# facebookresearch/generative-recommenders

Hardware: NVIDIA H100
Metric: user-seqs/sec HSTU-large L=8192 d=256 bf16 fwd+bwd (higher is better)
Workload: dtype bf16

## Files before the change

generative_recommenders_b200/_lib.py:

```python
import ctypes as C
import os
from typing import Optional

import torch

_HERE = os.path.dirname(os.path.abspath(__file__))
LIB_PATH = os.environ.get("HSTU_B200_LIB") or os.path.join(_HERE, "lib", "libhstu_b200.so")

ABI_VERSION = 1
F32, BF16, F16, E4M3 = 0, 1, 2, 3
IMPL_AUTO, IMPL_GENERIC, IMPL_UMMA = 0, 1, 2

_DTYPES = {torch.float32: F32, torch.bfloat16: BF16, torch.float16: F16, torch.float8_e4m3fn: E4M3}


class AttnParams(C.Structure):
    _fields_ = [
        ("abi_version", C.c_int32), ("dtype", C.c_int32), ("impl", C.c_int32), ("batch", C.c_int32),
        ("heads", C.c_int32), ("dqk", C.c_int32), ("dv", C.c_int32), ("max_seq_len", C.c_int32),
        ("total_rows", C.c_int64), ("alpha", C.c_float), ("max_attn_len", C.c_int32),
        ("min_full_attn_seq_len", C.c_int32), ("contextual_seq_len", C.c_int32), ("delta_q_len", C.c_int32),
        ("offsets_are_i64", C.c_int32), ("num_targets_are_i64", C.c_int32),
        ("seq_offsets", C.c_void_p), ("num_targets", C.c_void_p), ("q", C.c_void_p), ("k", C.c_void_p),
        ("v", C.c_void_p), ("out", C.c_void_p),
        ("q_row_stride", C.c_int64), ("q_head_stride", C.c_int64), ("k_row_stride", C.c_int64),
        ("k_head_stride", C.c_int64), ("v_row_stride", C.c_int64), ("v_head_stride", C.c_int64),
        ("o_row_stride", C.c_int64), ("o_head_stride", C.c_int64),
        ("dout", C.c_void_p), ("dq", C.c_void_p), ("dk", C.c_void_p), ("dv_out", C.c_void_p),
        ("do_row_stride", C.c_int64), ("do_head_stride", C.c_int64), ("dq_row_stride", C.c_int64),
        ("dq_head_stride", C.c_int64), ("dk_row_stride", C.c_int64), ("dk_head_stride", C.c_int64),
        ("dv_row_stride", C.c_int64), ("dv_head_stride", C.c_int64),
        ("pos_w", C.c_void_p), ("ts_w", C.c_void_p), ("timestamps", C.c_void_p), ("num_ts_buckets", C.c_int32),
        ("deterministic", C.c_int32), ("dpos_w", C.c_void_p), ("dts_w", C.c_void_p),
        ("workspace", C.c_void_p), ("workspace_bytes", C.c_size_t),
    ]


class Descales(C.Structure):
    _fields_ = [
        ("q", C.c_void_p), ("k", C.c_void_p), ("v", C.c_void_p),
        ("q_batch_stride", C.c_int64), ("q_head_stride", C.c_int64), ("k_batch_stride", C.c_int64),
        ("k_head_stride", C.c_int64), ("v_batch_stride", C.c_int64), ("v_head_stride", C.c_int64),
    ]


class SslParams(C.Structure):
    _fields_ = [
        ("abi_version", C.c_int32), ("dtype", C.c_int32), ("N", C.c_int64), ("R", C.c_int32), ("D", C.c_int32),
        ("l2_norm", C.c_int32), ("l2_eps", C.c_float), ("temperature", C.c_float), ("reserved0", C.c_int32),
        ("q", C.c_void_p), ("pos_emb", C.c_void_p), ("table", C.c_void_p), ("pos_ids", C.c_void_p), ("neg_ids", C.c_void_p),
        ("logits", C.c_void_p), ("rnorm", C.c_void_p), ("lse", C.c_void_p), ("loss_rows", C.c_void_p),
        ("row_coef", C.c_void_p), ("d_q", C.c_void_p), ("d_pos_emb", C.c_void_p), ("d_table", C.c_void_p),
    ]


_lib: Optional[C.CDLL] = None

_i32, _i64, _f32, _u64, _vp = C.c_int32, C.c_int64, C.c_float, C.c_uint64, C.c_void_p

_PROTOS = {
    "hstu_last_error": (C.c_char_p, []),
    "hstu_abi_version": (C.c_int, []),
    "hstu_attn_workspace_bytes": (C.c_size_t, [C.POINTER(AttnParams), C.c_int]),
    "hstu_attn_fwd": (C.c_int, [C.POINTER(AttnParams), _vp]),
    "hstu_attn_bwd": (C.c_int, [C.POINTER(AttnParams), _vp]),
    "hstu_attn_fwd_fp8": (C.c_int, [C.POINTER(AttnParams), C.POINTER(Descales), _vp]),
    "hstu_attn_select_impl": (C.c_int, [C.POINTER(AttnParams), C.c_int]),
    "hstu_mask_valid": (C.c_int, [_i32] * 7),
    "hstu_kv_range_for_q_rows": (C.c_int, [_i32] * 7 + [C.POINTER(_i32)] * 2),
    "hstu_q_range_for_kv_rows": (C.c_int, [_i32] * 7 + [C.POINTER(_i32)] * 3),
    "hstu_layer_norm_fwd": (C.c_int, [_vp, _vp, _vp, _vp, _vp, _vp, _i64, _i32, _i64, _i64, _f32, _i32, _i32, _vp]),
    "hstu_layer_norm_bwd": (C.c_int, [_vp] * 10 + [_i64, _i32, _i64, _i64, _i64, _i32, _i32, _vp]),
    "hstu_norm_bwd_partial_rows": (_i32, []),
    "hstu_rms_norm_fwd": (C.c_int, [_vp, _vp, _vp, _vp, _i64, _i32, _f32, _i32, _vp]),
    "hstu_rms_norm_bwd": (C.c_int, [_vp] * 7 + [_i64, _i32, _i32, _vp]),
    "hstu_norm_mul_dropout_fwd": (C.c_int, [_vp] * 7 + [_i64, _i32, _i32, _i64, _i64, _f32, _f32, _u64, _i32, _i32, _i32, _i32, _vp]),
    "hstu_norm_mul_dropout_bwd": (C.c_int, [_vp] * 12 + [_i64, _i32, _i32, _i64, _i64, _i64, _i64, _f32, _u64, _i32, _i32, _i32, _i32, _vp]),
    "hstu_silu_fwd": (C.c_int, [_vp, _vp, _i64, _i32, _i64, _i64, _i32, _vp]),
    "hstu_silu_bwd": (C.c_int, [_vp, _vp, _vp, _i64, _i32, _i64, _i64, _i64, _i32, _vp]),
    "hstu_jagged_concat": (C.c_int, [_vp] * 5 + [_i32] * 8 + [_vp]),
    "hstu_jagged_split": (C.c_int, [_vp] * 5 + [_i32] * 8 + [_vp]),
    "hstu_position_embeddings_fwd": (C.c_int, [_vp] * 10 + [_i64, _i32, _i32, _i32, _i32, _i32, _f32, _i32, _i32, _i32, _i32, _i32, _i32, _vp]),
    "hstu_position_embeddings_bwd": (C.c_int, [_vp] * 6 + [_i64, _i32, _f32, _i32, _vp]),
    "hstu_jagged_dense_bmm_broadcast_add": (C.c_int, [_vp] * 5 + [_i32] * 7 + [_vp]),
    "hstu_jagged_dense_bmm_wgrad": (C.c_int, [_vp] * 5 + [_i32] * 6 + [_vp]),
    "hstu_sampled_softmax_fwd": (C.c_int, [C.POINTER(SslParams), _vp]),
    "hstu_sampled_softmax_bwd": (C.c_int, [C.POINTER(SslParams), _vp]),
}

EXPORTED_SYMBOLS = tuple(_PROTOS.keys())


def lib() -> C.CDLL:
    global _lib
    if _lib is None:
        if not os.path.exists(LIB_PATH):
            raise RuntimeError(
                f"{LIB_PATH} is missing: build it with `python -m generative_recommenders_b200.build` "
                "(there is no CPU / eager fallback for HammerKernel.CUDA)"
            )
        l = C.CDLL(LIB_PATH)
        for name, (res, args) in _PROTOS.items():
            fn = getattr(l, name)
            fn.restype = res
            fn.argtypes = args
        if l.hstu_abi_version() != ABI_VERSION:
            raise RuntimeError("libhstu_b200.so ABI version mismatch")
        _lib = l
    return _lib


_selftest: Optional[C.CDLL] = None


def selftest_lib() -> C.CDLL:
    global _selftest
    if _selftest is None:
        path = os.path.join(_HERE, "lib", "libhstu_b200_selftest.so")
        if not os.path.exists(path):
            raise RuntimeError(f"{path} is missing: build it with `python -m generative_recommenders_b200.build`")
        l = C.CDLL(path)
        l.hstu_umma_selftest.restype = C.c_int
        l.hstu_umma_selftest.argtypes = [C.c_char_p, C.c_size_t]
        _selftest = l
    return _selftest


LAUNCHES = 0
_TIMED = None


def note_launch(n: int = 1) -> None:
    global LAUNCHES
    LAUNCHES += n


def enable_timing(on: bool) -> None:
    global _TIMED
    _TIMED = {} if on else None


def timed_events():
    return _TIMED


class timed:

    def __init__(self, name: str, device):
        self.name, self.device = name, device

    def __enter__(self):
        if _TIMED is not None:
            self.e0 = torch.cuda.Event(enable_timing=True)
            self.e1 = torch.cuda.Event(enable_timing=True)
            self.e0.record(torch.cuda.current_stream(self.device))
        return self

    def __exit__(self, *exc):
        if _TIMED is not None:
            self.e1.record(torch.cuda.current_stream(self.device))
            _TIMED.setdefault(self.name, []).append((self.e0, self.e1))
        return False


def check(rc: int, what: str) -> None:
    if rc != 0:
        msg = lib().hstu_last_error().decode(errors="replace")
        raise RuntimeError(f"{what} failed (code {rc}): {msg}")


def dtype_code(t: torch.Tensor) -> int:
    try:
        return _DTYPES[t.dtype]
    except KeyError:
        raise RuntimeError(f"unsupported dtype {t.dtype} for the CUDA HSTU kernels") from None


def ptr(t: Optional[torch.Tensor]) -> Optional[int]:
    return None if t is None else t.data_ptr()


def stream_ptr(device: torch.device) -> int:
    return torch.cuda.current_stream(device).cuda_stream


def require_cuda(*tensors: Optional[torch.Tensor]) -> torch.device:
    dev = None
    for t in tensors:
        if t is None:
            continue
        if not t.is_cuda:
            raise RuntimeError("HammerKernel.CUDA ops need CUDA tensors (no CPU fallback)")
        if dev is None:
            dev = t.device
        elif t.device != dev:
            raise RuntimeError("all tensors must be on the same CUDA device")
    assert dev is not None
    return dev
```

generative_recommenders_b200/csrc/api.cu:

```cuda
#include <stdarg.h>
#include <string.h>

#include "common.cuh"
#include "internal.h"

namespace hstu {

static thread_local char g_err[512] = "";

void set_error(const char* fmt, ...) {
  va_list ap;
  va_start(ap, fmt);
  vsnprintf(g_err, sizeof(g_err), fmt, ap);
  va_end(ap);
}

static int validate_attn(const hstu_attn_params* p, bool bwd) {
  HSTU_CHECK_ARG(p != nullptr, "params is NULL");
  HSTU_CHECK_ARG(p->abi_version == HSTU_B200_ABI_VERSION, "ABI version mismatch: caller %d, library %d", p->abi_version,
                 HSTU_B200_ABI_VERSION);
  HSTU_CHECK_ARG(p->dtype == HSTU_F32 || p->dtype == HSTU_BF16 || p->dtype == HSTU_F16 || p->dtype == HSTU_E4M3, "bad dtype %d",
                 p->dtype);
  HSTU_CHECK_ARG(p->max_seq_len > 0, "max_seq_len must be larger than 0");
  HSTU_CHECK_ARG(p->batch >= 0 && p->heads > 0, "bad batch/heads");
  HSTU_CHECK_ARG(p->dqk > 0 && p->dv > 0 && p->dqk <= 256 && p->dv <= 256, "head dims must be in [1, 256] (dqk=%d, dv=%d)",
                 p->dqk, p->dv);
  HSTU_CHECK_ARG(p->total_rows >= 0, "negative total_rows");
  HSTU_CHECK_ARG(p->max_attn_len >= 0 && p->contextual_seq_len >= 0 && p->min_full_attn_seq_len >= 0, "negative mask option");
  if (p->batch == 0 || p->total_rows == 0) return 0;
  HSTU_CHECK_ARG(p->seq_offsets != nullptr, "seq_offsets is NULL");
  HSTU_CHECK_ARG(p->q && p->k && p->v, "q/k/v is NULL");
  if (!bwd) HSTU_CHECK_ARG(p->out != nullptr, "out is NULL");
  if (bwd) {
    HSTU_CHECK_ARG(p->dout && p->dq && p->dk && p->dv_out, "dout/dq/dk/dv is NULL");
    HSTU_CHECK_ARG(p->delta_q_len == 0, "backward of delta-q attention is not defined by the reference");
  }
  if (p->ts_w) HSTU_CHECK_ARG(p->timestamps != nullptr, "ts_w given without timestamps");
  HSTU_CHECK_ARG(p->impl >= HSTU_IMPL_AUTO && p->impl <= HSTU_IMPL_UMMA, "bad impl %d", p->impl);
  HSTU_CHECK_ARG(p->deterministic == 0 || p->deterministic == 1, "deterministic must be 0 or 1 (got %d)", p->deterministic);
  return 0;
}

int bind_device(const void* ptr) {
  if (ptr == nullptr) return 0;
  cudaPointerAttributes attr;
  cudaError_t e = cudaPointerGetAttributes(&attr, ptr);
  if (e != cudaSuccess || (attr.type != cudaMemoryTypeDevice && attr.type != cudaMemoryTypeManaged)) {
    cudaGetLastError();
    set_error("expected a CUDA device pointer (got %p: %s)", ptr, e == cudaSuccess ? "host memory" : cudaGetErrorString(e));
    return HSTU_ERR_INVALID_ARGUMENT;
  }
  HSTU_CUDA_OK(cudaSetDevice(attr.device));
  return 0;
}

static int select_impl(const hstu_attn_params* p, bool bwd) {
  if (p->dtype == HSTU_E4M3) {
    if (bwd) {
      set_error("fp8 (e4m3) attention has no backward: hstu_attn_fwd_fp8 is a forward-only entry");
      return HSTU_ERR_UNSUPPORTED;
    }
    if (p->impl == HSTU_IMPL_GENERIC) {
      set_error("fp8 (e4m3) attention runs on the wgmma kernels only: the generic kernels take no fp8 input");
      return HSTU_ERR_UNSUPPORTED;
    }
    if (int e = e4m3_fwd_check(*p)) return e;
    return HSTU_IMPL_UMMA;
  }
  if (bwd && p->deterministic && (p->pos_w != nullptr || p->ts_w != nullptr)) {
    set_error("deterministic backward with a relative bias is not supported: the dpos_w / dts_w gradients are added "
              "with atomics");
    return HSTU_ERR_UNSUPPORTED;
  }
  const bool can = wgmma_supported(*p, bwd);
  if (p->impl == HSTU_IMPL_GENERIC) return HSTU_IMPL_GENERIC;
  if (p->impl == HSTU_IMPL_UMMA) {
    if (!can) {
      set_error("wgmma path does not support this problem (dtype=%d dqk=%d dv=%d delta=%d bias=%d)", p->dtype, p->dqk,
                p->dv, p->delta_q_len, p->pos_w != nullptr || p->ts_w != nullptr);
      return HSTU_ERR_UNSUPPORTED;
    }
    return HSTU_IMPL_UMMA;
  }
  return can ? HSTU_IMPL_UMMA : HSTU_IMPL_GENERIC;
}

static int validate_descales(const hstu_attn_descales* d) {
  if (d == nullptr) return 0;
  const float* ptr[3] = {d->q, d->k, d->v};
  const int64_t bs[3] = {d->q_batch_stride, d->k_batch_stride, d->v_batch_stride};
  const int64_t hs[3] = {d->q_head_stride, d->k_head_stride, d->v_head_stride};
  for (int i = 0; i < 3; ++i) {
    const char name = "qkv"[i];
    HSTU_CHECK_ARG(bs[i] >= 0 && hs[i] >= 0, "%c descale: negative stride (batch %lld, head %lld)", name, (long long)bs[i],
                   (long long)hs[i]);
    HSTU_CHECK_ARG((reinterpret_cast<uintptr_t>(ptr[i]) & 3) == 0, "%c descale: %p is not a float pointer", name, (const void*)ptr[i]);
  }
  return 0;
}

static int check_descale_devices(const hstu_attn_descales* d) {
  if (d == nullptr) return 0;
  int dev = 0;
  HSTU_CUDA_OK(cudaGetDevice(&dev));
  const float* ptr[3] = {d->q, d->k, d->v};
  for (int i = 0; i < 3; ++i) {
    if (ptr[i] == nullptr) continue;
    cudaPointerAttributes attr;
    const cudaError_t e = cudaPointerGetAttributes(&attr, ptr[i]);
    if (e != cudaSuccess || (attr.type != cudaMemoryTypeDevice && attr.type != cudaMemoryTypeManaged) || attr.device != dev) {
      cudaGetLastError();
      set_error("%c descale: expected device memory of CUDA device %d (got %p)", "qkv"[i], dev, (const void*)ptr[i]);
      return HSTU_ERR_INVALID_ARGUMENT;
    }
  }
  return 0;
}

}

using namespace hstu;

extern "C" {

const char* hstu_last_error(void) { return g_err; }
int hstu_abi_version(void) { return HSTU_B200_ABI_VERSION; }

int hstu_attn_select_impl(const hstu_attn_params* p, int is_backward) {
  if (int e = validate_attn(p, is_backward != 0)) return e;
  return select_impl(p, is_backward != 0);
}

size_t hstu_attn_workspace_bytes(const hstu_attn_params* p, int is_backward) {
  if (p == nullptr) return 0;
  if (validate_attn(p, is_backward != 0) != 0) return 0;
  if (p->batch == 0 || p->total_rows == 0) return 0;
  int impl = select_impl(p, is_backward != 0);
  if (p->dtype == HSTU_E4M3) return impl == HSTU_IMPL_UMMA ? e4m3_v_copy_bytes(*p) : 0;
  if (impl == HSTU_IMPL_UMMA) return wgmma_workspace_bytes(*p, is_backward != 0);
  return 0;
}

int hstu_attn_fwd(const hstu_attn_params* p, void* stream) {
  if (int e = validate_attn(p, false)) return e;
  HSTU_CHECK_ARG(p->dtype != HSTU_E4M3, "hstu_attn_fwd: fp8 (e4m3) inputs go through hstu_attn_fwd_fp8 (with their descales)");
  if (p->batch == 0 || p->total_rows == 0) return 0;
  if (int e = bind_device(p->q)) return e;
  int impl = select_impl(p, false);
  if (impl < 0) return impl;
  if (impl == HSTU_IMPL_UMMA) return attn_wgmma_fwd(*p, (cudaStream_t)stream);
  return attn_generic_fwd(*p, (cudaStream_t)stream);
}

int hstu_attn_bwd(const hstu_attn_params* p, void* stream) {
  if (int e = validate_attn(p, true)) return e;
  if (p->dtype == HSTU_E4M3) {
    set_error("hstu_attn_bwd: fp8 (e4m3) attention has no backward (hstu_attn_fwd_fp8 is forward only)");
    return HSTU_ERR_UNSUPPORTED;
  }
  if (p->batch == 0 || p->total_rows == 0) return 0;
  if (int e = bind_device(p->q)) return e;
  int impl = select_impl(p, true);
  if (impl < 0) return impl;
  if (impl == HSTU_IMPL_UMMA) return attn_wgmma_bwd(*p, (cudaStream_t)stream);
  return attn_generic_bwd(*p, (cudaStream_t)stream);
}

int hstu_attn_fwd_fp8(const hstu_attn_params* p, const hstu_attn_descales* descales, void* stream) {
  if (int e = validate_attn(p, false)) return e;
  HSTU_CHECK_ARG(p->dtype == HSTU_E4M3, "hstu_attn_fwd_fp8: q, k, v must be HSTU_E4M3 (got dtype %d)", p->dtype);
  if (int e = validate_descales(descales)) return e;
  const int impl = select_impl(p, false);
  if (impl < 0) return impl;
  if (p->batch == 0 || p->total_rows == 0) return 0;
  if (int e = bind_device(p->q)) return e;
  if (int e = check_descale_devices(descales)) return e;
  if (!is_sm90()) {
    set_error("hstu_attn_fwd_fp8: the fp8 kernels need an sm_90 device");
    return HSTU_ERR_UNSUPPORTED;
  }
  hstu_attn_descales none;
  memset(&none, 0, sizeof(none));
  return attn_wgmma_fwd_e4m3(*p, descales ? *descales : none, (cudaStream_t)stream);
}

int hstu_mask_valid(int32_t len, int32_t num_targets, int32_t max_attn_len, int32_t min_full_attn_seq_len,
                    int32_t contextual_seq_len, int32_t i, int32_t j) {
  SeqMask m = make_seq_mask(len, num_targets, max_attn_len, min_full_attn_seq_len, contextual_seq_len);
  return mask_valid(m, i, j) ? 1 : 0;
}

int hstu_kv_range_for_q_rows(int32_t len, int32_t num_targets, int32_t max_attn_len, int32_t min_full_attn_seq_len,
                             int32_t contextual_seq_len, int32_t m0, int32_t m1, int32_t* lo, int32_t* hi) {
  HSTU_CHECK_ARG(lo && hi && m0 >= 0 && m1 > m0 && m1 <= len, "bad row range");
  SeqMask m = make_seq_mask(len, num_targets, max_attn_len, min_full_attn_seq_len, contextual_seq_len);
  int l, h;
  kv_range_for_q_rows(m, m0, m1, &l, &h);
  *lo = l;
  *hi = h;
  return 0;
}

int hstu_q_range_for_kv_rows(int32_t len, int32_t num_targets, int32_t max_attn_len, int32_t min_full_attn_seq_len,
                             int32_t contextual_seq_len, int32_t n0, int32_t n1, int32_t* lo, int32_t* hi,
                             int32_t* ctx_hi) {
  HSTU_CHECK_ARG(lo && hi && ctx_hi && n0 >= 0 && n1 > n0 && n1 <= len, "bad row range");
  SeqMask m = make_seq_mask(len, num_targets, max_attn_len, min_full_attn_seq_len, contextual_seq_len);
  int l, h, c;
  q_range_for_kv_rows(m, n0, n1, &l, &h, &c);
  *lo = l;
  *hi = h;
  *ctx_hi = c;
  return 0;
}

int hstu_layer_norm_fwd(const void* x, const void* w, const void* b, void* y, float* mean, float* rstd, int64_t n_rows,
                        int32_t D, int64_t x_row_stride, int64_t y_row_stride, float eps, int32_t dtype, int32_t swish,
                        void* stream) {
  if (n_rows > 0) if (int e = bind_device(x)) return e;
  HSTU_CHECK_ARG(n_rows >= 0 && (n_rows == 0 || (x && y)), "layer_norm_fwd: NULL x/y");
  return layer_norm_fwd(x, w, b, y, mean, rstd, n_rows, D, x_row_stride, y_row_stride, eps, dtype, swish, false,
                        (cudaStream_t)stream);
}

int hstu_layer_norm_bwd(const void* dy, const void* x, const void* w, const void* b, const float* mean, const float* rstd,
                        void* dx, float* dw, float* db, float* partial, int64_t n_rows, int32_t D, int64_t x_row_stride,
                        int64_t dy_row_stride, int64_t dx_row_stride, int32_t dtype, int32_t swish, void* stream) {
  if (n_rows > 0) if (int e = bind_device(x)) return e;
  HSTU_CHECK_ARG(n_rows >= 0 && (n_rows == 0 || (dy && x && dx && mean && rstd)), "layer_norm_bwd: NULL argument");
  return layer_norm_bwd(dy, x, w, b, mean, rstd, dx, dw, db, partial, n_rows, D, x_row_stride, dy_row_stride,
                        dx_row_stride, dtype, swish, false, (cudaStream_t)stream);
}

int32_t hstu_norm_bwd_partial_rows(void) { return norm_partial_rows(); }

int hstu_rms_norm_fwd(const void* x, const void* w, void* y, float* rstd, int64_t n_rows, int32_t D, float eps,
                      int32_t dtype, void* stream) {
  if (n_rows > 0) if (int e = bind_device(x)) return e;
  HSTU_CHECK_ARG(n_rows >= 0 && (n_rows == 0 || (x && y && w)), "rms_norm_fwd: NULL argument");
  return layer_norm_fwd(x, w, nullptr, y, nullptr, rstd, n_rows, D, D, D, eps, dtype, 0, true, (cudaStream_t)stream);
}

int hstu_rms_norm_bwd(const void* dy, const void* x, const void* w, const float* rstd, void* dx, float* dw,
                      float* partial, int64_t n_rows, int32_t D, int32_t dtype, void* stream) {
  if (n_rows > 0) if (int e = bind_device(x)) return e;
  HSTU_CHECK_ARG(n_rows >= 0 && (n_rows == 0 || (dy && x && w && dx && rstd)), "rms_norm_bwd: NULL argument");
  return layer_norm_bwd(dy, x, w, nullptr, nullptr, rstd, dx, dw, nullptr, partial, n_rows, D, D, D, D, dtype, 0, true,
                        (cudaStream_t)stream);
}

int hstu_norm_mul_dropout_fwd(const void* attn, const void* u, const void* w, const void* b, void* out, float* mean,
                              float* rstd, int64_t n_rows, int32_t heads, int32_t dv, int64_t attn_row_stride,
                              int64_t u_row_stride, float eps, float dropout_p, uint64_t seed, int32_t dtype,
                              int32_t silu_u, int32_t concat_ux, int32_t group_norm, void* stream) {
  if (n_rows > 0) if (int e = bind_device(attn)) return e;
  HSTU_CHECK_ARG(n_rows >= 0 && (n_rows == 0 || (attn && u && w && b && out)), "norm_mul_dropout_fwd: NULL argument");
  HSTU_CHECK_ARG(dropout_p >= 0.f && dropout_p < 1.f, "dropout_p must be in [0, 1)");
  return norm_mul_dropout_fwd(attn, u, w, b, out, mean, rstd, n_rows, heads, dv, attn_row_stride, u_row_stride, eps,
                              dropout_p, seed, dtype, silu_u, concat_ux, group_norm, (cudaStream_t)stream);
}

int hstu_norm_mul_dropout_bwd(const void* dout, const void* attn, const void* u, const void* w, const void* b,
                              const float* mean, const float* rstd, void* dattn, void* du, float* dw, float* db,
                              float* partial, int64_t n_rows, int32_t heads, int32_t dv, int64_t attn_row_stride,
                              int64_t u_row_stride, int64_t dattn_row_stride, int64_t du_row_stride, float dropout_p,
                              uint64_t seed, int32_t dtype, int32_t silu_u, int32_t concat_ux, int32_t group_norm,
                              void* stream) {
  if (n_rows > 0) if (int e = bind_device(attn)) return e;
  HSTU_CHECK_ARG(n_rows >= 0 && (n_rows == 0 || (dout && attn && u && w && b && mean && rstd && dattn && du)),
                 "norm_mul_dropout_bwd: NULL argument");
  return norm_mul_dropout_bwd(dout, attn, u, w, b, mean, rstd, dattn, du, dw, db, partial, n_rows, heads, dv,
                              attn_row_stride, u_row_stride, dattn_row_stride, du_row_stride, dropout_p, seed, dtype,
                              silu_u, concat_ux, group_norm, (cudaStream_t)stream);
}

int hstu_silu_fwd(const void* x, void* y, int64_t n_rows, int32_t n_cols, int64_t x_row_stride, int64_t y_row_stride,
                  int32_t dtype, void* stream) {
  if (n_rows > 0) if (int e = bind_device(x)) return e;
  HSTU_CHECK_ARG(n_rows >= 0 && (n_rows == 0 || (x && y)), "silu_fwd: NULL argument");
  return silu_fwd_bwd(x, nullptr, y, n_rows, n_cols, x_row_stride, 0, y_row_stride, dtype, false, (cudaStream_t)stream);
}

int hstu_silu_bwd(const void* dy, const void* x, void* dx, int64_t n_rows, int32_t n_cols, int64_t dy_row_stride,
                  int64_t x_row_stride, int64_t dx_row_stride, int32_t dtype, void* stream) {
  if (n_rows > 0) if (int e = bind_device(x)) return e;
  HSTU_CHECK_ARG(n_rows >= 0 && (n_rows == 0 || (dy && x && dx)), "silu_bwd: NULL argument");
  return silu_fwd_bwd(x, dy, dx, n_rows, n_cols, x_row_stride, dy_row_stride, dx_row_stride, dtype, true,
                      (cudaStream_t)stream);
}

int hstu_jagged_concat(const void* left, const void* right, void* out, const void* offsets_left, const void* offsets_right,
                       int32_t offsets_are_i64, int32_t batch, int32_t dense_len_left, int32_t dense_len_right,
                       int32_t n_prefix, int32_t D, int32_t elem_bytes, int32_t max_seq_len, void* stream) {
  if (int e = bind_device(out)) return e;
  HSTU_CHECK_ARG(offsets_left || offsets_right, "offsets_left and offsets_right cannot be None at the same time");
  HSTU_CHECK_ARG(elem_bytes == 1 || elem_bytes == 2 || elem_bytes == 4 || elem_bytes == 8, "bad elem_bytes");
  return jagged_concat_split(false, left, right, out, nullptr, offsets_left, offsets_right, offsets_are_i64, batch,
                             dense_len_left, dense_len_right, n_prefix, D, elem_bytes, max_seq_len, (cudaStream_t)stream);
}

int hstu_jagged_split(const void* in, void* left, void* right, const void* offsets_left, const void* offsets_right,
                      int32_t offsets_are_i64, int32_t batch, int32_t dense_len_left, int32_t dense_len_right,
                      int32_t n_prefix, int32_t D, int32_t elem_bytes, int32_t max_seq_len, void* stream) {
  if (int e = bind_device(in)) return e;
  HSTU_CHECK_ARG(offsets_left || offsets_right, "offsets_left and offsets_right cannot be None at the same time");
  HSTU_CHECK_ARG(elem_bytes == 1 || elem_bytes == 2 || elem_bytes == 4 || elem_bytes == 8, "bad elem_bytes");
  return jagged_concat_split(true, in, nullptr, left, right, offsets_left, offsets_right, offsets_are_i64, batch,
                             dense_len_left, dense_len_right, n_prefix, D, elem_bytes, max_seq_len, (cudaStream_t)stream);
}

int hstu_position_embeddings_fwd(const void* seq_embeddings, void* out, const float* pos_w, const float* ts_w,
                                 const void* seq_offsets, const void* seq_lengths, const void* num_targets,
                                 const int64_t* timestamps, int32_t* pos_inds, int32_t* ts_inds, int64_t total_rows,
                                 int32_t batch, int32_t D, int32_t max_pos_ind, int32_t num_time_buckets,
                                 int32_t max_contextual_seq_len, float alpha, int32_t interleave_targets,
                                 int32_t log_time_bucket, int32_t offsets_are_i64, int32_t lengths_are_i64,
                                 int32_t num_targets_are_i64, int32_t dtype, void* stream) {
  HSTU_CHECK_ARG(total_rows >= 0 && batch >= 0 && D > 0, "position_embeddings_fwd: bad sizes");
  if (total_rows == 0) return 0;
  if (int e = bind_device(seq_embeddings)) return e;
  HSTU_CHECK_ARG(seq_embeddings && out && pos_w && ts_w && seq_offsets && seq_lengths && timestamps,
                 "position_embeddings_fwd: NULL argument");
  HSTU_CHECK_ARG(max_pos_ind > 0 && num_time_buckets >= 0, "position_embeddings_fwd: empty embedding table");
  PosArgs a;
  a.seq = seq_embeddings; a.out = out; a.pos_w = pos_w; a.ts_w = ts_w;
  a.seq_offsets = seq_offsets; a.seq_lengths = seq_lengths; a.num_targets = num_targets;
  a.timestamps = reinterpret_cast<const long long*>(timestamps);
  a.pos_inds = pos_inds; a.ts_inds = ts_inds;
  a.L = total_rows; a.B = batch; a.D = D;
  a.max_pos_ind = max_pos_ind; a.num_time_buckets = num_time_buckets; a.max_contextual = max_contextual_seq_len;
  a.offsets_i64 = offsets_are_i64; a.lengths_i64 = lengths_are_i64; a.targets_i64 = num_targets_are_i64;
  a.interleave = interleave_targets; a.log_bucket = log_time_bucket;
  a.vec_ok = (((uintptr_t)seq_embeddings | (uintptr_t)out | (uintptr_t)pos_w | (uintptr_t)ts_w) & 15) == 0;
  a.alpha = alpha;
  return position_fwd(a, dtype, (cudaStream_t)stream);
}

int hstu_position_embeddings_bwd(const void* dout, void* d_seq_embeddings, float* d_pos_w, float* d_ts_w,
                                 const int32_t* pos_inds, const int32_t* ts_inds, int64_t total_rows, int32_t D, float alpha,
                                 int32_t dtype, void* stream) {
  HSTU_CHECK_ARG(total_rows >= 0 && D > 0, "position_embeddings_bwd: bad sizes");
  if (total_rows == 0) return 0;
  if (int e = bind_device(dout)) return e;
  HSTU_CHECK_ARG(dout && d_seq_embeddings && d_pos_w && d_ts_w && pos_inds && ts_inds, "position_embeddings_bwd: NULL argument");
  return position_bwd(dout, d_seq_embeddings, d_pos_w, d_ts_w, pos_inds, ts_inds, total_rows, D, alpha, dtype, (cudaStream_t)stream);
}

int hstu_jagged_dense_bmm_broadcast_add(const void* jagged, const void* dense, const void* bias, void* out,
                                        const void* seq_offsets, int32_t offsets_are_i64, int32_t batch, int32_t K, int32_t N,
                                        int32_t max_seq_len, int32_t dense_is_transposed, int32_t dtype, void* stream) {
  HSTU_CHECK_ARG(batch >= 0 && K > 0 && N > 0 && max_seq_len > 0, "jagged_dense_bmm_broadcast_add: bad sizes");
  if (batch == 0) return 0;
  if (int e = bind_device(dense)) return e;
  HSTU_CHECK_ARG(dense && seq_offsets, "jagged_dense_bmm_broadcast_add: NULL argument");
  return jagged_bmm(jagged, dense, bias, out, seq_offsets, offsets_are_i64, batch, K, N, max_seq_len, dense_is_transposed != 0, dtype,
                    (cudaStream_t)stream);
}

int hstu_jagged_dense_bmm_wgrad(const void* jagged, const void* dout, void* d_dense, void* d_bias, const void* seq_offsets,
                                int32_t offsets_are_i64, int32_t batch, int32_t K, int32_t N, int32_t max_seq_len, int32_t dtype,
                                void* stream) {
  HSTU_CHECK_ARG(batch >= 0 && K > 0 && N > 0 && max_seq_len > 0, "jagged_dense_bmm_wgrad: bad sizes");
  if (batch == 0) return 0;
  if (int e = bind_device(d_dense)) return e;
  HSTU_CHECK_ARG(d_dense && seq_offsets, "jagged_dense_bmm_wgrad: NULL argument");
  return jagged_bmm_wgrad(jagged, dout, d_dense, d_bias, seq_offsets, offsets_are_i64, batch, K, N, max_seq_len, dtype,
                          (cudaStream_t)stream);
}

static int validate_ssl(const hstu_ssl_params* p, bool bwd) {
  HSTU_CHECK_ARG(p != nullptr, "params is NULL");
  HSTU_CHECK_ARG(p->abi_version == HSTU_B200_ABI_VERSION, "ABI version mismatch: caller %d, library %d", p->abi_version,
                 HSTU_B200_ABI_VERSION);
  HSTU_CHECK_ARG(p->N >= 0 && p->R >= 0 && p->D > 0, "sampled softmax: bad sizes");
  HSTU_CHECK_ARG(p->temperature > 0.f, "sampled softmax: temperature must be positive");
  if (p->N == 0) return 0;
  HSTU_CHECK_ARG(p->q && p->pos_emb && p->table && p->pos_ids && (p->neg_ids || p->R == 0), "sampled softmax: NULL input");
  HSTU_CHECK_ARG(p->logits && p->rnorm && p->lse, "sampled softmax: NULL logits / rnorm / lse");
  if (!bwd) HSTU_CHECK_ARG(p->loss_rows != nullptr, "sampled softmax: NULL loss_rows");
  if (bwd) HSTU_CHECK_ARG(p->row_coef && p->d_q && p->d_pos_emb && p->d_table, "sampled softmax backward: NULL argument");
  return 0;
}

int hstu_sampled_softmax_fwd(const hstu_ssl_params* p, void* stream) {
  if (int e = validate_ssl(p, false)) return e;
  if (p->N == 0) return 0;
  if (int e = bind_device(p->q)) return e;
  return sampled_softmax_fwd(*p, p->dtype, (cudaStream_t)stream);
}

int hstu_sampled_softmax_bwd(const hstu_ssl_params* p, void* stream) {
  if (int e = validate_ssl(p, true)) return e;
  if (p->N == 0) return 0;
  if (int e = bind_device(p->q)) return e;
  return sampled_softmax_bwd(*p, p->dtype, (cudaStream_t)stream);
}


}
```

generative_recommenders_b200/csrc/attn_fp16_operands.cu:

```cuda
#include <cuda_fp16.h>
#include <cuda_fp8.h>
#include <string.h>

#include "attn_fp16_operands.cuh"
#include "common.cuh"
#include "internal.h"

namespace hstu {

constexpr int kPreRows = 256, kPreThreads = 256, kPreD = 32;

struct PreOperand {
  const void* src;
  long long row_stride, head_stride;
  __half* dst;
};

struct PreParams {
  PreOperand op[kAmaxSlots];
  int nops;
  const void* seq_offsets;
  int offsets_i64, max_seq_len, heads;
  int d;
  float alpha;
  uint32_t* amax;
};

__device__ __forceinline__ float bf16_bits_to_float(uint32_t b) { return __uint_as_float(b << 16); }

__global__ void __launch_bounds__(kPreThreads) fp16_operands_amax_kernel(const __grid_constant__ PreParams p) {
  const int b = blockIdx.z, h = blockIdx.y;
  const long long row0 = load_index(p.seq_offsets, p.offsets_i64, b);
  const int len = min((int)(load_index(p.seq_offsets, p.offsets_i64, b + 1) - row0), p.max_seq_len);
  const int r0 = blockIdx.x * kPreRows;
  if (r0 >= len) return;
  const int rows = min(kPreRows, len - r0);
  __shared__ uint32_t red[kAmaxSlots][kPreThreads / 32];
  const int warp = threadIdx.x >> 5, lane = threadIdx.x & 31;
  for (int o = 0; o < p.nops; ++o) {
    const PreOperand& op = p.op[o];
    uint32_t m = 0u;
    for (int c = threadIdx.x; c < rows * 4; c += kPreThreads) {
      const int r = c >> 2, part = c & 3;
      const uint4 x = *reinterpret_cast<const uint4*>(reinterpret_cast<const uint16_t*>(op.src) + (row0 + r0 + r) * op.row_stride +
                                                      (long long)h * op.head_stride + part * 8);
      const uint32_t w[4] = {x.x, x.y, x.z, x.w};
#pragma unroll
      for (int i = 0; i < 4; ++i) {
        m = max(m, (w[i] & 0x7fffu) << 16);
        m = max(m, (w[i] >> 16 & 0x7fffu) << 16);
      }
    }
#pragma unroll
    for (int s = 16; s > 0; s >>= 1) m = max(m, __shfl_xor_sync(0xffffffffu, m, s));
    if (lane == 0) red[o][warp] = m;
  }
  __syncthreads();
  if (threadIdx.x < p.nops) {
    uint32_t m = 0u;
#pragma unroll
    for (int w = 0; w < kPreThreads / 32; ++w) m = max(m, red[threadIdx.x][w]);
    if (m) atomicMax(p.amax + ((long long)b * p.heads + h) * kAmaxSlots + threadIdx.x, m);
  }
}

template <bool E4M3>
__global__ void __launch_bounds__(kPreThreads) fp16_operands_convert_kernel(const __grid_constant__ PreParams p) {
  const int b = blockIdx.z, h = blockIdx.y;
  const long long row0 = load_index(p.seq_offsets, p.offsets_i64, b);
  const int len = min((int)(load_index(p.seq_offsets, p.offsets_i64, b + 1) - row0), p.max_seq_len);
  const int r0 = blockIdx.x * kPreRows;
  if (r0 >= len) return;
  const int rows = min(kPreRows, len - r0);
  const int d = E4M3 ? p.d : kPreD, cpr = d / 8;
  int exps[kAmaxSlots] = {0, 0, 0, 0};
  if constexpr (!E4M3) {
    const OperandExps ex = operand_exps(p.amax + ((long long)b * p.heads + h) * kAmaxSlots, p.alpha, kPreD);
    exps[0] = ex.q, exps[1] = ex.k, exps[2] = ex.v, exps[3] = ex.o;
  }
  for (int o = 0; o < p.nops; ++o) {
    const PreOperand& op = p.op[o];
    const int e = exps[o];
    for (int c = threadIdx.x; c < rows * cpr; c += kPreThreads) {
      const int r = c / cpr, part = c % cpr;
      const long long row = row0 + r0 + r;
      uint32_t y[4];
      if constexpr (E4M3) {
        const uint2 x = *reinterpret_cast<const uint2*>(reinterpret_cast<const uint8_t*>(op.src) + row * op.row_stride +
                                                        (long long)h * op.head_stride + part * 8);
        const uint32_t w[2] = {x.x, x.y};
#pragma unroll
        for (int i = 0; i < 4; ++i) {
          const __half2_raw v = __nv_cvt_fp8x2_to_halfraw2((__nv_fp8x2_storage_t)(w[i >> 1] >> (16 * (i & 1))), __NV_E4M3);
          y[i] = (uint32_t)v.x | ((uint32_t)v.y << 16);
        }
      } else {
        const uint4 x = *reinterpret_cast<const uint4*>(reinterpret_cast<const uint16_t*>(op.src) + row * op.row_stride +
                                                        (long long)h * op.head_stride + part * 8);
        const uint32_t w[4] = {x.x, x.y, x.z, x.w};
#pragma unroll
        for (int i = 0; i < 4; ++i) {
          const __half2 v = __floats2half2_rn(scalbnf(bf16_bits_to_float(w[i] & 0xffffu), e), scalbnf(bf16_bits_to_float(w[i] >> 16), e));
          y[i] = *reinterpret_cast<const uint32_t*>(&v);
        }
      }
      *reinterpret_cast<uint4*>(op.dst + (row * p.heads + h) * d + part * 8) = make_uint4(y[0], y[1], y[2], y[3]);
    }
  }
}

static size_t align256(size_t n) { return (n + 255) / 256 * 256; }

size_t fp16_operands_workspace_bytes(const hstu_attn_params& p, bool bwd) {
  const size_t amax = align256((size_t)p.batch * p.heads * kAmaxSlots * sizeof(uint32_t));
  const size_t copy = align256((size_t)p.total_rows * p.heads * kPreD * sizeof(__half));
  return amax + (bwd ? 4 : 3) * copy;
}

int fp16_operands_prepass(const hstu_attn_params& p, bool bwd, Fp16Operands* out, cudaStream_t st) {
  const size_t need = fp16_operands_workspace_bytes(p, bwd);
  if (p.workspace == nullptr || p.workspace_bytes < need) {
    set_error("hstu_attn_%s: workspace of %zu bytes required (got %zu)", bwd ? "bwd" : "fwd", need, p.workspace_bytes);
    return HSTU_ERR_WORKSPACE;
  }
  uint8_t* ws = reinterpret_cast<uint8_t*>(p.workspace);
  const size_t amax_bytes = (size_t)p.batch * p.heads * kAmaxSlots * sizeof(uint32_t);
  const size_t copy = align256((size_t)p.total_rows * p.heads * kPreD * sizeof(__half));
  PreParams pp;
  memset(&pp, 0, sizeof(pp));
  pp.amax = reinterpret_cast<uint32_t*>(ws);
  const void* src[kAmaxSlots] = {p.q, p.k, p.v, p.dout};
  const long long rs[kAmaxSlots] = {p.q_row_stride, p.k_row_stride, p.v_row_stride, p.do_row_stride};
  const long long hs[kAmaxSlots] = {p.q_head_stride, p.k_head_stride, p.v_head_stride, p.do_head_stride};
  pp.nops = bwd ? 4 : 3;
  for (int o = 0; o < pp.nops; ++o) {
    pp.op[o].src = src[o];
    pp.op[o].row_stride = rs[o];
    pp.op[o].head_stride = hs[o];
    pp.op[o].dst = reinterpret_cast<__half*>(ws + align256(amax_bytes) + o * copy);
    out->copy[o] = pp.op[o].dst;
  }
  out->amax = pp.amax;
  pp.seq_offsets = p.seq_offsets;
  pp.offsets_i64 = p.offsets_are_i64;
  pp.max_seq_len = p.max_seq_len;
  pp.heads = p.heads;
  pp.alpha = p.alpha;
  HSTU_CUDA_OK(cudaMemsetAsync(pp.amax, 0, amax_bytes, st));
  if (p.batch == 0 || p.max_seq_len <= 0) return 0;
  const dim3 grid((p.max_seq_len + kPreRows - 1) / kPreRows, p.heads, p.batch);
  fp16_operands_amax_kernel<<<grid, kPreThreads, 0, st>>>(pp);
  HSTU_CUDA_OK(cudaGetLastError());
  fp16_operands_convert_kernel<false><<<grid, kPreThreads, 0, st>>>(pp);
  HSTU_CUDA_OK(cudaGetLastError());
  return 0;
}

size_t e4m3_v_copy_bytes(const hstu_attn_params& p) { return align256((size_t)p.total_rows * p.heads * p.dv * sizeof(__half)); }

int e4m3_v_prepass(const hstu_attn_params& p, const void** v16, cudaStream_t st) {
  const size_t need = e4m3_v_copy_bytes(p);
  if (p.workspace == nullptr || p.workspace_bytes < need) {
    set_error("hstu_attn_fwd_fp8: workspace of %zu bytes required (got %zu)", need, p.workspace_bytes);
    return HSTU_ERR_WORKSPACE;
  }
  PreParams pp;
  memset(&pp, 0, sizeof(pp));
  pp.nops = 1;
  pp.op[0].src = p.v;
  pp.op[0].row_stride = p.v_row_stride;
  pp.op[0].head_stride = p.v_head_stride;
  pp.op[0].dst = reinterpret_cast<__half*>(p.workspace);
  *v16 = p.workspace;
  pp.seq_offsets = p.seq_offsets;
  pp.offsets_i64 = p.offsets_are_i64;
  pp.max_seq_len = p.max_seq_len;
  pp.heads = p.heads;
  pp.d = p.dv;
  if (p.batch == 0 || p.max_seq_len <= 0) return 0;
  const dim3 grid((p.max_seq_len + kPreRows - 1) / kPreRows, p.heads, p.batch);
  fp16_operands_convert_kernel<true><<<grid, kPreThreads, 0, st>>>(pp);
  HSTU_CUDA_OK(cudaGetLastError());
  return 0;
}

}
```

generative_recommenders_b200/csrc/attn_wgmma_bwd.cu:

```cuda
#include "attn_wgmma_bwd.cuh"

namespace hstu {

template <int D, bool BF16>
__global__ void __launch_bounds__(kAttnThreads, 1) attn_bwd_wgmma_kernel(const __grid_constant__ BwdParams p) {
  bwd_key_tile<D, D, BF16, true>(p);
}

template <int D, bool BF16>
__global__ void __launch_bounds__(kAttnThreads, split_min_blocks(D)) attn_bwd_dkdv_wgmma_kernel(const __grid_constant__ BwdParams p) {
  bwd_key_tile<D, D, BF16, false>(p);
}

template <int D, bool BF16>
__global__ void __launch_bounds__(kAttnThreads, split_min_blocks(D)) attn_bwd_dq_wgmma_kernel(const __grid_constant__ BwdParams p) {
  bwd_dq_body<D, D, BF16>(p);
}

template <bool BF16>
__global__ void dq_convert_kernel(const float* __restrict__ acc, uint16_t* __restrict__ dq, long long rows, int heads, int D,
                                  long long row_stride, long long head_stride, float scale) {
  const long long nvec = rows * heads * (D / 8);
  for (long long idx = (long long)blockIdx.x * blockDim.x + threadIdx.x; idx < nvec; idx += (long long)gridDim.x * blockDim.x) {
    const int v = (int)(idx % (D / 8));
    const long long rh = idx / (D / 8);
    const int hh = (int)(rh % heads);
    const long long r = rh / heads;
    const float4 a = *reinterpret_cast<const float4*>(acc + rh * D + v * 8);
    const float4 c = *reinterpret_cast<const float4*>(acc + rh * D + v * 8 + 4);
    uint4 o;
    if (BF16) {
      o = make_uint4(pack_bf16x2(a.x * scale, a.y * scale), pack_bf16x2(a.z * scale, a.w * scale),
                     pack_bf16x2(c.x * scale, c.y * scale), pack_bf16x2(c.z * scale, c.w * scale));
    } else {
      o = make_uint4(pack_f16x2(a.x * scale, a.y * scale), pack_f16x2(a.z * scale, a.w * scale),
                     pack_f16x2(c.x * scale, c.y * scale), pack_f16x2(c.z * scale, c.w * scale));
    }
    *reinterpret_cast<uint4*>(dq + r * row_stride + hh * head_stride + v * 8) = o;
  }
}

static bool wgmma_bwd_supported(const hstu_attn_params& p) {
  if (!wgmma_fwd_supported(p)) return false;
  if ((p.dqk == 256 || p.dqk != p.dv) && p.deterministic) return false;
  return aligned_view(p.dout, p.do_row_stride, p.do_head_stride) && aligned_view(p.dq, p.dq_row_stride, p.dq_head_stride) &&
         aligned_view(p.dk, p.dk_row_stride, p.dk_head_stride) && aligned_view(p.dv_out, p.dv_row_stride, p.dv_head_stride);
}

bool wgmma_supported(const hstu_attn_params& p, bool bwd) {
  if (!bwd) return wgmma_fwd_supported(p);
  hstu_attn_params q = p;
  if (q.out == nullptr) q.out = const_cast<void*>(q.q);
  q.o_row_stride = 8;
  q.o_head_stride = 8;
  return wgmma_bwd_supported(q);
}

static bool split_dq(const hstu_attn_params& p) {
  return p.dqk == 32 || p.dqk == 256 || p.dqk != p.dv || p.deterministic != 0;
}

static bool fp16_copies(const hstu_attn_params& p) { return p.dtype == HSTU_BF16 && p.dqk == 32 && p.dv == 32; }

size_t wgmma_workspace_bytes(const hstu_attn_params& p, bool bwd) {
  if (!bwd && p.delta_q_len > 0) return wgmma_delta_workspace_bytes(p);
  if (fp16_copies(p)) return fp16_operands_workspace_bytes(p, bwd);
  if (!bwd || split_dq(p)) return 0;
  return (size_t)p.total_rows * p.heads * p.dqk * sizeof(float);
}

template <int D, bool BF16, bool kSplit>
static int launch_bwd_wgmma(const hstu_attn_params& p, cudaStream_t st, const Fp16Operands* f16 = nullptr) {
  if constexpr (kSplit) {
    return launch_bwd_split<D, D, BF16>(p, st, attn_bwd_dkdv_wgmma_kernel<D, BF16>, attn_bwd_dq_wgmma_kernel<D, BF16>, f16);
  } else {
    using Cfg = BwdCfg<D, D, true>;
    const size_t need = wgmma_workspace_bytes(p, true);
    if (p.workspace == nullptr || p.workspace_bytes < need) {
      set_error("hstu_attn_bwd: workspace of %zu bytes required (got %zu)", need, p.workspace_bytes);
      return HSTU_ERR_WORKSPACE;
    }
    const BwdOperands o = bwd_operands(p, f16);
    BwdParams bp = bwd_params(p, f16);
    if (int e = make_tmap_rows_heads(&bp.tmQ, o.src[0], p.total_rows, p.heads, D, o.rs[0], o.hs[0], Cfg::BOX_COLS, Cfg::BQ)) return e;
    if (int e = make_tmap_rows_heads(&bp.tmK, o.src[1], p.total_rows, p.heads, D, o.rs[1], o.hs[1], Cfg::BOX_COLS, Cfg::BKV)) return e;
    if (int e = make_tmap_rows_heads(&bp.tmV, o.src[2], p.total_rows, p.heads, D, o.rs[2], o.hs[2], Cfg::BOX_COLS, Cfg::BKV)) return e;
    if (int e = make_tmap_rows_heads(&bp.tmDO, o.src[3], p.total_rows, p.heads, D, o.rs[3], o.hs[3], Cfg::BOX_COLS, Cfg::BQ)) return e;
    HSTU_CUDA_OK(cudaMemsetAsync(p.workspace, 0, need, st));
    auto kern = attn_bwd_wgmma_kernel<D, BF16>;
    HSTU_CUDA_OK(cudaFuncSetAttribute(kern, cudaFuncAttributeMaxDynamicSharedMemorySize, Cfg::SMEM_BYTES));
    dim3 grid((p.max_seq_len + Cfg::BKV - 1) / Cfg::BKV, p.heads, p.batch);
    kern<<<grid, kAttnThreads, Cfg::SMEM_BYTES, st>>>(bp);
    HSTU_CUDA_OK(cudaGetLastError());
    const long long nvec = p.total_rows * p.heads * (D / 8);
    long long blocks = (nvec + 255) / 256;
    if (blocks > 132 * 16) blocks = 132 * 16;
    dq_convert_kernel<BF16><<<(int)blocks, 256, 0, st>>>(bp.dq_acc, reinterpret_cast<uint16_t*>(p.dq), p.total_rows, p.heads, D,
                                                         p.dq_row_stride, p.dq_head_stride, bp.dk_scale);
    HSTU_CUDA_OK(cudaGetLastError());
    return 0;
  }
}

int attn_wgmma_bwd(const hstu_attn_params& p, cudaStream_t st) {
  if (p.dqk != p.dv) return attn_wgmma_bwd_mixed(p, st);
  const bool bf = p.dtype == HSTU_BF16;
  const bool split = split_dq(p);
  switch (p.dqk) {
    case 32: {
      if (!bf) return launch_bwd_wgmma<32, false, true>(p, st);
      Fp16Operands f16;
      if (int e = fp16_operands_prepass(p, true, &f16, st)) return e;
      return launch_bwd_wgmma<32, false, true>(p, st, &f16);
    }
    case 64:
      if (split) return bf ? launch_bwd_wgmma<64, true, true>(p, st) : launch_bwd_wgmma<64, false, true>(p, st);
      return bf ? launch_bwd_wgmma<64, true, false>(p, st) : launch_bwd_wgmma<64, false, false>(p, st);
    case 128:
      if (split) return bf ? launch_bwd_wgmma<128, true, true>(p, st) : launch_bwd_wgmma<128, false, true>(p, st);
      return bf ? launch_bwd_wgmma<128, true, false>(p, st) : launch_bwd_wgmma<128, false, false>(p, st);
    case 256:
      return bf ? launch_bwd_wgmma<256, true, true>(p, st) : launch_bwd_wgmma<256, false, true>(p, st);
  }
  set_error("wgmma backward: unsupported head dim %d", p.dqk);
  return HSTU_ERR_UNSUPPORTED;
}

}
```

generative_recommenders_b200/csrc/attn_wgmma_fwd.cu:

```cuda
#include "attn_wgmma_fwd.cuh"

namespace hstu {

template <int D, bool BF16>
__global__ void __launch_bounds__(kAttnThreads, kFwdMinBlocks<D>) attn_fwd_wgmma_kernel(const __grid_constant__ FwdParams p) {
  attn_fwd_wgmma_body<D, D, BF16, false>(p);
}
template <int D, bool BF16>
__global__ void __launch_bounds__(kAttnThreads, kFwdMinBlocks<D>) attn_fwd_delta_wgmma_kernel(const __grid_constant__ FwdParams p) {
  attn_fwd_wgmma_body<D, D, BF16, true>(p);
}

template <bool BF16>
__global__ void __launch_bounds__(256) delta_reduce_kernel(const float* __restrict__ part, void* out, long long rows, int heads, int d,
                                                            int chunks, long long o_row_stride, long long o_head_stride, float inv_n) {
  const long long plane = rows * heads * d, n4 = plane / 4;
  for (long long i = (long long)blockIdx.x * 256 + threadIdx.x; i < n4; i += (long long)gridDim.x * 256) {
    float4 a = reinterpret_cast<const float4*>(part)[i];
    for (int c = 1; c < chunks; ++c) {
      const float4 x = reinterpret_cast<const float4*>(part + c * plane)[i];
      a.x += x.x, a.y += x.y, a.z += x.z, a.w += x.w;
    }
    const long long e = i * 4, r = e / ((long long)heads * d), hc = e % ((long long)heads * d);
    const long long off = r * o_row_stride + (hc / d) * o_head_stride + hc % d;
    a.x *= inv_n, a.y *= inv_n, a.z *= inv_n, a.w *= inv_n;
    const uint2 v = BF16 ? make_uint2(pack_bf16x2(a.x, a.y), pack_bf16x2(a.z, a.w)) : make_uint2(pack_f16x2(a.x, a.y), pack_f16x2(a.z, a.w));
    *reinterpret_cast<uint2*>(reinterpret_cast<uint16_t*>(out) + off) = v;
  }
}

constexpr int kH100Sms = 132;
constexpr int kDeltaCtaTarget = 2 * kH100Sms, kDeltaChunkKeys = 512;
constexpr int kDeltaReduceBlocks = 8 * kH100Sms;
int delta_chunks(const hstu_attn_params& p) {
  const long long ctas = (long long)p.batch * p.heads * ((p.delta_q_len + FwdCfg<32>::BM - 1) / FwdCfg<32>::BM);
  if (ctas >= kDeltaCtaTarget) return 1;
  const long long by_len = ((long long)p.max_seq_len + kDeltaChunkKeys - 1) / kDeltaChunkKeys;
  return (int)std::max(1ll, std::min(by_len, kDeltaCtaTarget / ctas));
}

size_t wgmma_delta_workspace_bytes(const hstu_attn_params& p) {
  const int c = delta_chunks(p);
  return c > 1 ? (size_t)c * p.batch * p.delta_q_len * p.heads * p.dv * sizeof(float) : 0;
}

bool is_sm90() {
  static int cached = -1;
  if (cached < 0) {
    int dev = 0;
    cudaDeviceProp prop;
    cached = (cudaGetDevice(&dev) == cudaSuccess && cudaGetDeviceProperties(&prop, dev) == cudaSuccess && prop.major == 9) ? 1 : 0;
  }
  return cached == 1;
}

bool aligned_view(const void* ptr, long long row_stride, long long head_stride) {
  return (reinterpret_cast<uintptr_t>(ptr) & 15) == 0 && (row_stride % 8) == 0 && (head_stride % 8) == 0;
}

bool wgmma_fwd_supported(const hstu_attn_params& p) {
  if (p.dtype != HSTU_BF16 && p.dtype != HSTU_F16) return false;
  auto dim_ok = [](int d) { return d == 32 || d == 64 || d == 128 || d == 256; };
  if (p.dqk > p.dv || !dim_ok(p.dqk) || !dim_ok(p.dv)) return false;
  if (p.delta_q_len < 0 || p.pos_w != nullptr || p.ts_w != nullptr) return false;
  if (p.total_rows >= (1ll << 31) - 256 || (long long)p.batch * p.delta_q_len >= (1ll << 31) - 256) return false;
  if (!aligned_view(p.q, p.q_row_stride, p.q_head_stride) || !aligned_view(p.k, p.k_row_stride, p.k_head_stride) ||
      !aligned_view(p.v, p.v_row_stride, p.v_head_stride) || !aligned_view(p.out, p.o_row_stride, p.o_head_stride))
    return false;
  return is_sm90();
}

int launch_delta_reduce(bool bf16, const float* part, void* out, long long rows, int heads, int d, int chunks,
                        long long o_row_stride, long long o_head_stride, float inv_n, cudaStream_t st) {
  const long long n4 = rows * heads * d / 4;
  const int blocks = (int)std::min<long long>((n4 + 255) / 256, kDeltaReduceBlocks);
  auto kern = bf16 ? delta_reduce_kernel<true> : delta_reduce_kernel<false>;
  kern<<<blocks, 256, 0, st>>>(part, out, rows, heads, d, chunks, o_row_stride, o_head_stride, inv_n);
  HSTU_CUDA_OK(cudaGetLastError());
  return 0;
}

template <int D, bool BF16, bool kDelta = false>
static int launch_fwd(const hstu_attn_params& p, cudaStream_t st, const Fp16Operands* f16 = nullptr) {
  auto kern = [] {
    if constexpr (kDelta) return attn_fwd_delta_wgmma_kernel<D, BF16>;
    else return attn_fwd_wgmma_kernel<D, BF16>;
  }();
  return launch_fwd_wgmma<D, D, BF16, kDelta>(p, st, kern, f16);
}

int attn_wgmma_fwd(const hstu_attn_params& p, cudaStream_t st) {
  if (p.dqk != p.dv) return attn_wgmma_fwd_mixed(p, st);
  const bool bf = p.dtype == HSTU_BF16;
  if (p.delta_q_len > 0) {
    switch (p.dqk) {
      case 32: return bf ? launch_fwd<32, true, true>(p, st) : launch_fwd<32, false, true>(p, st);
      case 64: return bf ? launch_fwd<64, true, true>(p, st) : launch_fwd<64, false, true>(p, st);
      case 128: return bf ? launch_fwd<128, true, true>(p, st) : launch_fwd<128, false, true>(p, st);
      case 256: return bf ? launch_fwd<256, true, true>(p, st) : launch_fwd<256, false, true>(p, st);
    }
  }
  switch (p.dqk) {
    case 32: {
      if (!bf) return launch_fwd<32, false>(p, st);
      Fp16Operands f16;
      if (int e = fp16_operands_prepass(p, false, &f16, st)) return e;
      return launch_fwd<32, false>(p, st, &f16);
    }
    case 64: return bf ? launch_fwd<64, true>(p, st) : launch_fwd<64, false>(p, st);
    case 128: return bf ? launch_fwd<128, true>(p, st) : launch_fwd<128, false>(p, st);
    case 256: return bf ? launch_fwd<256, true>(p, st) : launch_fwd<256, false>(p, st);
  }
  set_error("wgmma forward: unsupported head dim %d", p.dqk);
  return HSTU_ERR_UNSUPPORTED;
}

}
```

generative_recommenders_b200/csrc/internal.h:

```cpp
#pragma once
#include <cuda_runtime.h>
#include <stddef.h>

#include "../../include/hstu_b200.h"

namespace hstu {
void set_error(const char* fmt, ...);

int attn_generic_fwd(const hstu_attn_params& p, cudaStream_t st);
int attn_generic_bwd(const hstu_attn_params& p, cudaStream_t st);

bool wgmma_supported(const hstu_attn_params& p, bool bwd);
size_t wgmma_workspace_bytes(const hstu_attn_params& p, bool bwd);
int attn_wgmma_fwd(const hstu_attn_params& p, cudaStream_t st);
int attn_wgmma_bwd(const hstu_attn_params& p, cudaStream_t st);
int attn_wgmma_fwd_mixed(const hstu_attn_params& p, cudaStream_t st);
int attn_wgmma_bwd_mixed(const hstu_attn_params& p, cudaStream_t st);
bool aligned_view(const void* ptr, long long row_stride, long long head_stride);
bool wgmma_fwd_supported(const hstu_attn_params& p);
size_t wgmma_delta_workspace_bytes(const hstu_attn_params& p);

struct Fp16Operands {
  const unsigned int* amax;
  const void* copy[4];
};
size_t fp16_operands_workspace_bytes(const hstu_attn_params& p, bool bwd);
int fp16_operands_prepass(const hstu_attn_params& p, bool bwd, Fp16Operands* out, cudaStream_t st);
size_t e4m3_v_copy_bytes(const hstu_attn_params& p);
int e4m3_v_prepass(const hstu_attn_params& p, const void** v16, cudaStream_t st);

int e4m3_fwd_check(const hstu_attn_params& p);
int attn_wgmma_fwd_e4m3(const hstu_attn_params& p, const hstu_attn_descales& ds, cudaStream_t st);
int attn_wgmma_fwd_e4m3_mixed(const hstu_attn_params& p, const hstu_attn_descales& ds, const void* v16, cudaStream_t st);
bool is_sm90();

int layer_norm_fwd(const void* x, const void* w, const void* b, void* y, float* mean, float* rstd, long long n, int D,
                   long long xs, long long ys, float eps, int dtype, int swish, bool rms, cudaStream_t st);
int layer_norm_bwd(const void* dy, const void* x, const void* w, const void* b, const float* mean, const float* rstd,
                   void* dx, float* dw, float* db, float* partial, long long n, int D, long long xs, long long dys,
                   long long dxs, int dtype, int swish, bool rms, cudaStream_t st);
int norm_mul_dropout_fwd(const void* attn, const void* u, const void* w, const void* b, void* out, float* mean,
                         float* rstd, long long n, int H, int dv, long long as, long long us, float eps, float p,
                         unsigned long long seed, int dtype, int silu_u, int concat, int gn, cudaStream_t st);
int norm_mul_dropout_bwd(const void* dout, const void* attn, const void* u, const void* w, const void* b,
                         const float* mean, const float* rstd, void* dattn, void* du, float* dw, float* db,
                         float* partial, long long n, int H, int dv, long long as, long long us, long long das,
                         long long dus, float p, unsigned long long seed, int dtype, int silu_u, int concat, int gn,
                         cudaStream_t st);
int silu_fwd_bwd(const void* x, const void* dy, void* out, long long n, int cols, long long xs, long long dys,
                 long long os, int dtype, bool bwd, cudaStream_t st);
int norm_partial_rows();

struct PosArgs {
  const void* seq;
  void* out;
  const float* pos_w;
  const float* ts_w;
  const void* seq_offsets;
  const void* seq_lengths;
  const void* num_targets;
  const long long* timestamps;
  int* pos_inds;
  int* ts_inds;
  long long L;
  int B, D;
  int max_pos_ind, num_time_buckets, max_contextual;
  int offsets_i64, lengths_i64, targets_i64;
  int interleave, log_bucket, vec_ok;
  float alpha;
};
int position_fwd(const PosArgs& a, int dtype, cudaStream_t st);
int position_bwd(const void* dout, void* dseq, float* dpos, float* dts, const int* pos_inds, const int* ts_inds, long long L, int D,
                 float alpha, int dtype, cudaStream_t st);

typedef hstu_ssl_params SslArgs;
int sampled_softmax_fwd(const SslArgs& a, int dtype, cudaStream_t st);
int sampled_softmax_bwd(const SslArgs& a, int dtype, cudaStream_t st);

int jagged_bmm(const void* A, const void* Bm, const void* bias, void* C, const void* off, int off_i64, int batch, int K, int N,
               int max_seq_len, bool trans_b, int dtype, cudaStream_t st);
int jagged_bmm_wgrad(const void* A, const void* G, void* dW, void* dbias, const void* off, int off_i64, int batch, int K, int N,
                     int max_seq_len, int dtype, cudaStream_t st);

int jagged_concat_split(bool split, const void* a, const void* b, void* c, void* c2, const void* off_l, const void* off_r,
                        int is_i64, int batch, int dense_l, int dense_r, int n_prefix, int D, int elem_bytes,
                        int max_seq_len, cudaStream_t st);
}
```

generative_recommenders_b200/csrc/norm.cu:

```cuda
#include "common.cuh"

namespace hstu {

bool norm_fast_applicable(int dtype, int len);
int layer_norm_fwd_fast(const void* x, const void* w, const void* b, void* y, float* mean, float* rstd, long long n, long long xs,
                        long long ys, float eps, int dtype, cudaStream_t st);
int layer_norm_bwd_fast(const void* dy, const void* x, const void* w, const float* mean, const float* rstd, void* dx, float* partial,
                        long long n, long long xs, long long dys, long long dxs, int dtype, int* grid_out, cudaStream_t st);
int norm_mul_dropout_fwd_fast(const void* attn, const void* u, const void* w, const void* b, void* out, float* mean, float* rstd,
                              long long n, long long as, long long us, float eps, float p, unsigned long long seed, int dtype,
                              int silu_u, int concat, cudaStream_t st);
int norm_mul_dropout_bwd_fast(const void* dout, const void* attn, const void* u, const void* w, const void* b, const float* mean,
                              const float* rstd, void* dattn, void* du, float* partial, long long n, long long as, long long us,
                              long long das, long long dus, float p, unsigned long long seed, int dtype, int silu_u, int concat,
                              int* grid_out, cudaStream_t st);

constexpr int kNormThreads = 256;
constexpr int kNormWarps = kNormThreads / 32;
constexpr int kMaxPerLane = 32;
constexpr int kPartialRows = 528;
constexpr int kFwdGridCap = 2112;

__device__ __forceinline__ float warp_sum(float v) {
#pragma unroll
  for (int o = 16; o > 0; o >>= 1) v += __shfl_xor_sync(0xffffffffu, v, o);
  return v;
}

template <typename T, int VEC, int PL>
struct RowIO {
  static __device__ __forceinline__ void load(const T* row, int D, int lane, float (&v)[PL]) {
#pragma unroll
    for (int k = 0; k < PL / VEC; ++k) {
      const int c = (k * 32 + lane) * VEC;
      if (c < D) {
        if constexpr (VEC == 1) {
          v[k] = Cvt<T>::to_f(row[c]);
        } else {
          uint4 raw = *reinterpret_cast<const uint4*>(row + c);
          const T* e = reinterpret_cast<const T*>(&raw);
#pragma unroll
          for (int i = 0; i < VEC; ++i) v[k * VEC + i] = Cvt<T>::to_f(e[i]);
        }
      } else {
#pragma unroll
        for (int i = 0; i < VEC; ++i) v[k * VEC + i] = 0.f;
      }
    }
  }
  static __device__ __forceinline__ void prefetch(const T* row, int D, int lane) {
#ifdef HSTU_NORM_NO_PREFETCH
    return;
#endif
    if constexpr (VEC > 1) {
#pragma unroll
      for (int k = 0; k < PL / VEC; ++k) {
        const int c = (k * 32 + lane) * VEC;
        if (c < D) asm volatile("prefetch.global.L2 [%0];" ::"l"(row + c));
      }
    }
  }
  static __device__ __forceinline__ void store(T* row, int D, int lane, const float (&v)[PL]) {
#pragma unroll
    for (int k = 0; k < PL / VEC; ++k) {
      const int c = (k * 32 + lane) * VEC;
      if (c < D) {
        if constexpr (VEC == 1) {
          row[c] = Cvt<T>::from_f(v[k]);
        } else {
          uint4 raw;
          T* e = reinterpret_cast<T*>(&raw);
#pragma unroll
          for (int i = 0; i < VEC; ++i) e[i] = Cvt<T>::from_f(v[k * VEC + i]);
          *reinterpret_cast<uint4*>(row + c) = raw;
        }
      }
    }
  }
};

#define FOR_OWNED(VEC, D, lane, k, i, c)                  \
  _Pragma("unroll") for (int k = 0; k < PL / VEC; ++k) \
  _Pragma("unroll") for (int i = 0; i < VEC; ++i)         \
    if (int c = (k * 32 + lane) * VEC + i; c < D)

__device__ __forceinline__ unsigned long long dropout_hash4(unsigned long long seed, unsigned long long idx4) {
  unsigned long long z = seed + 0x9E3779B97F4A7C15ull * (idx4 + 1);
  z = (z ^ (z >> 30)) * 0xBF58476D1CE4E5B9ull;
  z = (z ^ (z >> 27)) * 0x94D049BB133111EBull;
  return z ^ (z >> 31);
}
__device__ __forceinline__ uint32_t dropout_threshold(float p) {
  const float t = p * 65536.0f + 0.5f;
  return t >= 65536.f ? 65536u : (uint32_t)t;
}
__device__ __forceinline__ bool dropout_keep(unsigned long long seed, unsigned long long idx, uint32_t thr) {
  const unsigned long long z = dropout_hash4(seed, idx >> 2);
  return (uint32_t)((z >> (16 * (idx & 3))) & 0xffffu) >= thr;
}
template <int VEC, int PL>
__device__ __forceinline__ void apply_dropout(float (&v)[PL], int len, int lane, unsigned long long base,
                                              unsigned long long seed, uint32_t thr, float keep_scale) {
  if constexpr (VEC % 4 == 0) {
#pragma unroll
    for (int k = 0; k < PL / VEC; ++k) {
      const int c0 = (k * 32 + lane) * VEC;
      if (c0 < len) {
#pragma unroll
        for (int g = 0; g < VEC / 4; ++g) {
          const unsigned long long z = dropout_hash4(seed, (base + c0 + g * 4) >> 2);
#pragma unroll
          for (int e = 0; e < 4; ++e) {
            const bool keep = (uint32_t)((z >> (16 * e)) & 0xffffu) >= thr;
            v[k * VEC + g * 4 + e] = keep ? v[k * VEC + g * 4 + e] * keep_scale : 0.f;
          }
        }
      }
    }
  } else {
#pragma unroll
    for (int k = 0; k < PL / VEC; ++k)
#pragma unroll
      for (int i = 0; i < VEC; ++i) {
        const int c = (k * 32 + lane) * VEC + i;
        if (c < len) v[k * VEC + i] = dropout_keep(seed, base + c, thr) ? v[k * VEC + i] * keep_scale : 0.f;
      }
  }
}

template <typename T, int VEC, int PL, bool RMS>
__global__ void __launch_bounds__(kNormThreads) ln_fwd_kernel(const T* __restrict__ x, const T* __restrict__ w,
                                                               const T* __restrict__ b, T* __restrict__ y,
                                                               float* __restrict__ mean_out, float* __restrict__ rstd_out,
                                                               long long n_rows, int D, long long xs, long long ys,
                                                               float eps, int swish) {
  const int lane = threadIdx.x & 31, warp = threadIdx.x >> 5;
  float wv[PL], bv[PL];
  if (w) RowIO<T, VEC, PL>::load(w, D, lane, wv);
  if (b) RowIO<T, VEC, PL>::load(b, D, lane, bv);
  const float inv_d = 1.0f / (float)D;
  const long long rstep = (long long)gridDim.x * kNormWarps;
  for (long long r = (long long)blockIdx.x * kNormWarps + warp; r < n_rows; r += rstep) {
    float v[PL];
    if (r + rstep < n_rows) RowIO<T, VEC, PL>::prefetch(x + (r + rstep) * xs, D, lane);
    RowIO<T, VEC, PL>::load(x + r * xs, D, lane, v);
    float mean = 0.f;
    if constexpr (!RMS) {
      float s = 0.f;
#pragma unroll
      for (int i = 0; i < PL; ++i) s += v[i];
      mean = warp_sum(s) * inv_d;
    }
    float s2 = 0.f;
    FOR_OWNED(VEC, D, lane, k, i, c) {
      const float dlt = v[k * VEC + i] - mean;
      s2 += dlt * dlt;
    }
    const float rstd = rsqrtf(warp_sum(s2) * inv_d + eps);
    float o[PL];
#pragma unroll
    for (int i = 0; i < PL; ++i) {
      float z = (v[i] - mean) * rstd;
      if (w) z *= wv[i];
      if (b) z += bv[i];
      o[i] = swish ? v[i] * sigmoid_f(z) : z;
    }
    RowIO<T, VEC, PL>::store(y + r * ys, D, lane, o);
    if (lane == 0) {
      if (mean_out) mean_out[r] = mean;
      if (rstd_out) rstd_out[r] = rstd;
    }
  }
}

template <typename T, int VEC, int PL, bool RMS>
__global__ void __launch_bounds__(kNormThreads) ln_bwd_kernel(const T* __restrict__ dy, const T* __restrict__ x,
                                                               const T* __restrict__ w, const T* __restrict__ b,
                                                               const float* __restrict__ mean_in,
                                                               const float* __restrict__ rstd_in, T* __restrict__ dx,
                                                               float* __restrict__ partial, long long n_rows, int D,
                                                               long long xs, long long dys, long long dxs, int swish) {
  extern __shared__ float red[];
  const int lane = threadIdx.x & 31, warp = threadIdx.x >> 5;
  float wv[PL], bv[PL];
  if (w) RowIO<T, VEC, PL>::load(w, D, lane, wv);
  if (b) RowIO<T, VEC, PL>::load(b, D, lane, bv);
  float aw[PL], ab[PL];
#pragma unroll
  for (int i = 0; i < PL; ++i) aw[i] = ab[i] = 0.f;
  const float inv_d = 1.0f / (float)D;
  const long long rstep = (long long)gridDim.x * kNormWarps;
  for (long long r = (long long)blockIdx.x * kNormWarps + warp; r < n_rows; r += rstep) {
    float xv[PL], g[PL];
    if (r + rstep < n_rows) {
      RowIO<T, VEC, PL>::prefetch(x + (r + rstep) * xs, D, lane);
      RowIO<T, VEC, PL>::prefetch(dy + (r + rstep) * dys, D, lane);
    }
    RowIO<T, VEC, PL>::load(x + r * xs, D, lane, xv);
    RowIO<T, VEC, PL>::load(dy + r * dys, D, lane, g);
    const float mean = RMS ? 0.f : mean_in[r];
    const float rstd = rstd_in[r];
    float direct[PL];
    float c1 = 0.f, c2 = 0.f;
#pragma unroll
    for (int i = 0; i < PL; ++i) {
      const float xhat = (xv[i] - mean) * rstd;
      float dz = g[i];
      direct[i] = 0.f;
      if (swish) {
        float z = xhat;
        if (w) z *= wv[i];
        if (b) z += bv[i];
        const float sg = sigmoid_f(z);
        direct[i] = g[i] * sg;
        dz = g[i] * xv[i] * sg * (1.f - sg);
      }
      aw[i] += dz * xhat;
      ab[i] += dz;
      const float wdy = w ? dz * wv[i] : dz;
      g[i] = wdy;
      c1 += xhat * wdy;
      c2 += wdy;
      xv[i] = xhat;
    }
    c1 = warp_sum(c1) * inv_d;
    c2 = RMS ? 0.f : warp_sum(c2) * inv_d;
    float o[PL];
#pragma unroll
    for (int i = 0; i < PL; ++i) o[i] = (g[i] - (xv[i] * c1 + c2)) * rstd + direct[i];
    RowIO<T, VEC, PL>::store(dx + r * dxs, D, lane, o);
  }
  if (partial == nullptr) return;
  FOR_OWNED(VEC, D, lane, k, i, c) {
    red[(warp * 2 + 0) * D + c] = aw[k * VEC + i];
    red[(warp * 2 + 1) * D + c] = ab[k * VEC + i];
  }
  __syncthreads();
  for (int c = threadIdx.x; c < 2 * D; c += kNormThreads) {
    float s = 0.f;
#pragma unroll
    for (int wp = 0; wp < kNormWarps; ++wp) s += red[wp * 2 * D + c];
    partial[(long long)blockIdx.x * 2 * D + c] = s;
  }
}

constexpr int kColsumGroups = 32;
__global__ void __launch_bounds__(32 * kColsumGroups) colsum_kernel(const float* __restrict__ partial, int rows, int ncols,
                                                                    int split, float* out0, float* out1) {
  __shared__ float red[kColsumGroups][33];
  const int lane = threadIdx.x & 31, g = threadIdx.x >> 5;
  const int c = blockIdx.x * 32 + lane;
  float s = 0.f;
  if (c < ncols) {
#pragma unroll 4
    for (int r = g; r < rows; r += kColsumGroups) s += partial[(long long)r * ncols + c];
  }
  red[g][lane] = s;
  __syncthreads();
  if (g == 0 && c < ncols) {
    float t = 0.f;
#pragma unroll
    for (int k = 0; k < kColsumGroups; ++k) t += red[k][lane];
    if (c < split) {
      if (out0) out0[c] = t;
    } else {
      if (out1) out1[c - split] = t;
    }
  }
}

template <typename T, int VEC, int PL>
__global__ void __launch_bounds__(kNormThreads) nmd_fwd_kernel(const T* __restrict__ attn, const T* __restrict__ u,
                                                                const T* __restrict__ w, const T* __restrict__ b,
                                                                T* __restrict__ out, float* __restrict__ mean_out,
                                                                float* __restrict__ rstd_out, long long n_rows, int G,
                                                                int len, long long as, long long us, float eps, float p,
                                                                unsigned long long seed, int silu_u, int concat,
                                                                int group_norm) {
  const int lane = threadIdx.x & 31, warp = threadIdx.x >> 5;
  const int width = G * len;
  const long long os = (long long)(concat ? 3 : 1) * width;
  float wv[PL], bv[PL];
  if (!group_norm) {
    RowIO<T, VEC, PL>::load(w, len, lane, wv);
    RowIO<T, VEC, PL>::load(b, len, lane, bv);
  }
  const float inv_d = 1.0f / (float)len;
  const float keep_scale = p > 0.f ? 1.0f / (1.0f - p) : 1.0f;
  const uint32_t thr = dropout_threshold(p);
  const long long n_vec = n_rows * G;
  const long long vstep = (long long)gridDim.x * kNormWarps;
  for (long long vi = (long long)blockIdx.x * kNormWarps + warp; vi < n_vec; vi += vstep) {
    const long long r = vi / G;
    const int gidx = (int)(vi - r * G);
    float a[PL], uu[PL];
    if (vi + vstep < n_vec) {
      const long long r2 = (vi + vstep) / G;
      const int g2 = (int)(vi + vstep - r2 * G);
      RowIO<T, VEC, PL>::prefetch(attn + r2 * as + g2 * len, len, lane);
      RowIO<T, VEC, PL>::prefetch(u + r2 * us + g2 * len, len, lane);
    }
    RowIO<T, VEC, PL>::load(attn + r * as + gidx * len, len, lane, a);
    RowIO<T, VEC, PL>::load(u + r * us + gidx * len, len, lane, uu);
    float s = 0.f;
#pragma unroll
    for (int i = 0; i < PL; ++i) s += a[i];
    const float mean = warp_sum(s) * inv_d;
    float s2 = 0.f;
    FOR_OWNED(VEC, len, lane, k, i, c) {
      const float dlt = a[k * VEC + i] - mean;
      s2 += dlt * dlt;
    }
    const float rstd = rsqrtf(warp_sum(s2) * inv_d + eps);
    float gw = 1.f, gb = 0.f;
    if (group_norm) {
      gw = Cvt<T>::to_f(w[gidx]);
      gb = Cvt<T>::to_f(b[gidx]);
    }
    float y[PL];
#pragma unroll
    for (int i = 0; i < PL; ++i) {
      if (silu_u) uu[i] = silu_f(uu[i]);
      const float xhat = (a[i] - mean) * rstd;
      const float nrm = group_norm ? xhat * gw + gb : xhat * wv[i] + bv[i];
      y[i] = uu[i] * nrm;
      if (concat == 2) a[i] = nrm;
    }
    T* orow = out + r * os + gidx * len;
    if (p > 0.f) {
      const unsigned long long base = (unsigned long long)r * os + gidx * len;
      if (concat) {
        apply_dropout<VEC, PL>(uu, len, lane, base, seed, thr, keep_scale);
        apply_dropout<VEC, PL>(a, len, lane, base + width, seed, thr, keep_scale);
        apply_dropout<VEC, PL>(y, len, lane, base + 2 * width, seed, thr, keep_scale);
      } else {
        apply_dropout<VEC, PL>(y, len, lane, base, seed, thr, keep_scale);
      }
    }
    if (concat) {
      RowIO<T, VEC, PL>::store(orow, len, lane, uu);
      RowIO<T, VEC, PL>::store(orow + width, len, lane, a);
      RowIO<T, VEC, PL>::store(orow + 2 * width, len, lane, y);
    } else {
      RowIO<T, VEC, PL>::store(orow, len, lane, y);
    }
    if (lane == 0) {
      if (mean_out) mean_out[vi] = mean;
      if (rstd_out) rstd_out[vi] = rstd;
    }
  }
}

template <typename T, int VEC, int PL>
__global__ void __launch_bounds__(kNormThreads) nmd_bwd_kernel(
    const T* __restrict__ dout, const T* __restrict__ attn, const T* __restrict__ u, const T* __restrict__ w,
    const T* __restrict__ b, const float* __restrict__ mean_in, const float* __restrict__ rstd_in, T* __restrict__ dattn,
    T* __restrict__ du, float* __restrict__ partial, long long n_rows, int G, int len, long long as, long long us,
    long long das, long long dus, float p, unsigned long long seed, int silu_u, int concat, int group_norm) {
  extern __shared__ float red[];
  const int lane = threadIdx.x & 31, warp = threadIdx.x >> 5;
  const int width = G * len;
  const long long os = (long long)(concat ? 3 : 1) * width;
  float wv[PL], bv[PL];
  float aw[PL], ab[PL];
#pragma unroll
  for (int i = 0; i < PL; ++i) aw[i] = ab[i] = 0.f;
  if (!group_norm) {
    RowIO<T, VEC, PL>::load(w, len, lane, wv);
    RowIO<T, VEC, PL>::load(b, len, lane, bv);
  } else {
    for (int c = threadIdx.x; c < kNormWarps * 2 * G; c += kNormThreads) red[c] = 0.f;
    __syncthreads();
  }
  const float inv_d = 1.0f / (float)len;
  const float keep_scale = p > 0.f ? 1.0f / (1.0f - p) : 1.0f;
  const uint32_t thr = dropout_threshold(p);
  const long long n_vec = n_rows * G;
  const long long vstep = (long long)gridDim.x * kNormWarps;
  for (long long vi = (long long)blockIdx.x * kNormWarps + warp; vi < n_vec; vi += vstep) {
    const long long r = vi / G;
    const int gidx = (int)(vi - r * G);
    float a[PL], uu[PL], gy[PL], gu[PL], ga[PL];
    if (vi + vstep < n_vec) {
      const long long r2 = (vi + vstep) / G;
      const int g2 = (int)(vi + vstep - r2 * G);
      RowIO<T, VEC, PL>::prefetch(attn + r2 * as + g2 * len, len, lane);
      RowIO<T, VEC, PL>::prefetch(u + r2 * us + g2 * len, len, lane);
      const T* d2 = dout + r2 * os + g2 * len;
      RowIO<T, VEC, PL>::prefetch(d2, len, lane);
      if (concat) {
        RowIO<T, VEC, PL>::prefetch(d2 + width, len, lane);
        RowIO<T, VEC, PL>::prefetch(d2 + 2 * width, len, lane);
      }
    }
    RowIO<T, VEC, PL>::load(attn + r * as + gidx * len, len, lane, a);
    RowIO<T, VEC, PL>::load(u + r * us + gidx * len, len, lane, uu);
    const T* drow = dout + r * os + gidx * len;
    if (concat) {
      RowIO<T, VEC, PL>::load(drow, len, lane, gu);
      RowIO<T, VEC, PL>::load(drow + width, len, lane, ga);
      RowIO<T, VEC, PL>::load(drow + 2 * width, len, lane, gy);
    } else {
      RowIO<T, VEC, PL>::load(drow, len, lane, gy);
#pragma unroll
      for (int i = 0; i < PL; ++i) gu[i] = ga[i] = 0.f;
    }
    if (p > 0.f) {
      const unsigned long long base = (unsigned long long)r * os + gidx * len;
      if (concat) {
        apply_dropout<VEC, PL>(gu, len, lane, base, seed, thr, keep_scale);
        apply_dropout<VEC, PL>(ga, len, lane, base + width, seed, thr, keep_scale);
        apply_dropout<VEC, PL>(gy, len, lane, base + 2 * width, seed, thr, keep_scale);
      } else {
        apply_dropout<VEC, PL>(gy, len, lane, base, seed, thr, keep_scale);
      }
    }
    const float mean = mean_in[vi], rstd = rstd_in[vi];
    float gw = 1.f, gb = 0.f;
    if (group_norm) {
      gw = Cvt<T>::to_f(w[gidx]);
      gb = Cvt<T>::to_f(b[gidx]);
    }
    float c1 = 0.f, c2 = 0.f, sgw = 0.f, sgb = 0.f;
#pragma unroll
    for (int i = 0; i < PL; ++i) {
      const float g_mid = concat == 2 ? ga[i] : 0.f;
      if (concat == 2) ga[i] = 0.f;
      const float upre = uu[i];
      float sg = 0.f;
      float ua = upre;
      if (silu_u) {
        sg = sigmoid_f(upre);
        ua = upre * sg;
      }
      const float xhat = (a[i] - mean) * rstd;
      const float wi = group_norm ? gw : wv[i];
      const float nrm = xhat * wi + (group_norm ? gb : bv[i]);
      float dua = gy[i] * nrm + gu[i];
      const float dn = gy[i] * ua + g_mid;
      if (silu_u) dua *= sg * (1.f + upre * (1.f - sg));
      gu[i] = dua;
      if (group_norm) {
        sgw += dn * xhat;
        sgb += dn;
      } else {
        aw[i] += dn * xhat;
        ab[i] += dn;
      }
      const float wdy = dn * wi;
      gy[i] = wdy;
      c1 += xhat * wdy;
      c2 += wdy;
      a[i] = xhat;
    }
    c1 = warp_sum(c1) * inv_d;
    c2 = warp_sum(c2) * inv_d;
#pragma unroll
    for (int i = 0; i < PL; ++i) ga[i] += (gy[i] - (a[i] * c1 + c2)) * rstd;
    RowIO<T, VEC, PL>::store(dattn + r * das + gidx * len, len, lane, ga);
    RowIO<T, VEC, PL>::store(du + r * dus + gidx * len, len, lane, gu);
    if (group_norm) {
      sgw = warp_sum(sgw);
      sgb = warp_sum(sgb);
      if (lane == 0) {
        red[(warp * 2 + 0) * G + gidx] += sgw;
        red[(warp * 2 + 1) * G + gidx] += sgb;
      }
    }
  }
  if (partial == nullptr) return;
  const int np = group_norm ? G : len;
  if (!group_norm) {
    FOR_OWNED(VEC, len, lane, k, i, c) {
      red[(warp * 2 + 0) * len + c] = aw[k * VEC + i];
      red[(warp * 2 + 1) * len + c] = ab[k * VEC + i];
    }
  }
  __syncthreads();
  for (int c = threadIdx.x; c < 2 * np; c += kNormThreads) {
    float s = 0.f;
#pragma unroll
    for (int wp = 0; wp < kNormWarps; ++wp) s += red[wp * 2 * np + c];
    partial[(long long)blockIdx.x * 2 * np + c] = s;
  }
}

template <typename T, int VEC, bool BWD>
__global__ void silu_kernel(const T* __restrict__ x, const T* __restrict__ dy, T* __restrict__ out, long long n_rows,
                            int n_cols, long long xs, long long dys, long long os) {
  constexpr int U = (VEC == 1 || BWD) ? 1 : 4;
  const int vec_per_row = n_cols / VEC;
  const long long total = n_rows * vec_per_row;
  const long long stride = blockDim.x;
  const long long chunk = (long long)blockDim.x * U;
  for (long long idx0 = (long long)blockIdx.x * chunk + threadIdx.x; idx0 - threadIdx.x < total; idx0 += (long long)gridDim.x * chunk) {
    T xv[U][VEC], gv[U][VEC];
    long long xo[U], oo[U];
#pragma unroll
    for (int k = 0; k < U; ++k) {
      const long long idx = idx0 + k * stride;
      if (idx < total) {
        const long long r = idx / vec_per_row;
        const int c = (int)(idx - r * vec_per_row) * VEC;
        xo[k] = r * xs + c;
        oo[k] = r * os + c;
        if constexpr (VEC == 1) {
          xv[k][0] = x[xo[k]];
          if (BWD) gv[k][0] = dy[r * dys + c];
        } else {
          *reinterpret_cast<uint4*>(xv[k]) = *reinterpret_cast<const uint4*>(x + xo[k]);
          if (BWD) *reinterpret_cast<uint4*>(gv[k]) = *reinterpret_cast<const uint4*>(dy + r * dys + c);
        }
      }
    }
#pragma unroll
    for (int k = 0; k < U; ++k) {
      if (idx0 + k * stride < total) {
        T ov[VEC];
#pragma unroll
        for (int i = 0; i < VEC; ++i) {
          const float xf = Cvt<T>::to_f(xv[k][i]);
          const float sg = sigmoid_f(xf);
          float o = xf * sg;
          if (BWD) o = Cvt<T>::to_f(gv[k][i]) * sg * (1.f + xf * (1.f - sg));
          ov[i] = Cvt<T>::from_f(o);
        }
        if constexpr (VEC == 1) {
          out[oo[k]] = ov[0];
        } else {
          *reinterpret_cast<uint4*>(out + oo[k]) = *reinterpret_cast<const uint4*>(ov);
        }
      }
    }
  }
}

static inline bool aligned16(const void* p) { return p == nullptr || (reinterpret_cast<uintptr_t>(p) & 15) == 0; }

static inline int norm_grid(long long n_vec, bool fwd = false) {
  long long need = (n_vec + kNormWarps - 1) / kNormWarps;
  if (need < 1) need = 1;
  const int cap = fwd ? kFwdGridCap : kPartialRows;
  return (int)(need < cap ? need : cap);
}

static bool fast_layout(std::initializer_list<const void*> ptrs, std::initializer_list<long long> strides) {
#ifdef HSTU_NORM_NO_FAST
  return false;
#endif
  for (const void* p : ptrs)
    if (p == nullptr || !aligned16(p)) return false;
  for (long long s : strides)
    if (s % 8) return false;
  return true;
}

template <typename T>
static bool can_vec(int D, std::initializer_list<const void*> ptrs, std::initializer_list<long long> strides) {
  constexpr int VEC = 16 / sizeof(T);
  if (D % VEC) return false;
  for (const void* p : ptrs)
    if (!aligned16(p)) return false;
  for (long long s : strides)
    if (s % VEC) return false;
  return true;
}

template <typename T, typename F>
static int dispatch_shape(int D, bool vec, F&& f) {
  constexpr int V = 16 / sizeof(T);
  if (D <= 256) return vec ? f.template operator()<V, 8>() : f.template operator()<1, 8>();
  if (D <= 512) return vec ? f.template operator()<V, 16>() : f.template operator()<1, 16>();
  return vec ? f.template operator()<V, 32>() : f.template operator()<1, 32>();
}

template <typename T>
static int ln_fwd_t(const void* x, const void* w, const void* b, void* y, float* mean, float* rstd, long long n, int D,
                    long long xs, long long ys, float eps, int swish, bool rms, cudaStream_t st) {
  const bool v = can_vec<T>(D, {x, w, b, y}, {xs, ys});
  const int grid = norm_grid(n, true);
  return dispatch_shape<T>(D, v, [&]<int VV, int PL>() -> int {
    if (rms)
      ln_fwd_kernel<T, VV, PL, true><<<grid, kNormThreads, 0, st>>>((const T*)x, (const T*)w, (const T*)b, (T*)y, mean,
                                                                    rstd, n, D, xs, ys, eps, swish);
    else
      ln_fwd_kernel<T, VV, PL, false><<<grid, kNormThreads, 0, st>>>((const T*)x, (const T*)w, (const T*)b, (T*)y, mean,
                                                                     rstd, n, D, xs, ys, eps, swish);
    HSTU_CUDA_OK(cudaGetLastError());
    return 0;
  });
}

template <typename T>
static int ln_bwd_t(const void* dy, const void* x, const void* w, const void* b, const float* mean, const float* rstd,
                    void* dx, float* dw, float* db, float* partial, long long n, int D, long long xs, long long dys,
                    long long dxs, int swish, bool rms, cudaStream_t st) {
  const bool v = can_vec<T>(D, {dy, x, w, b, dx}, {xs, dys, dxs});
  const int grid = norm_grid(n);
  const bool want_param = (dw != nullptr || db != nullptr);
  if (want_param && partial == nullptr) {
    set_error("layer_norm_bwd: dw/db requested but no partial scratch given");
    return HSTU_ERR_WORKSPACE;
  }
  float* part = want_param ? partial : nullptr;
  const size_t smem = sizeof(float) * kNormWarps * 2 * (size_t)D;
  int rc = dispatch_shape<T>(D, v, [&]<int VV, int PL>() -> int {
    if (rms) {
      HSTU_CUDA_OK(cudaFuncSetAttribute(ln_bwd_kernel<T, VV, PL, true>, cudaFuncAttributeMaxDynamicSharedMemorySize, (int)smem));
      ln_bwd_kernel<T, VV, PL, true><<<grid, kNormThreads, smem, st>>>((const T*)dy, (const T*)x, (const T*)w, (const T*)b,
                                                                       mean, rstd, (T*)dx, part, n, D, xs, dys, dxs, swish);
    } else {
      HSTU_CUDA_OK(cudaFuncSetAttribute(ln_bwd_kernel<T, VV, PL, false>, cudaFuncAttributeMaxDynamicSharedMemorySize, (int)smem));
      ln_bwd_kernel<T, VV, PL, false><<<grid, kNormThreads, smem, st>>>((const T*)dy, (const T*)x, (const T*)w, (const T*)b,
                                                                        mean, rstd, (T*)dx, part, n, D, xs, dys, dxs, swish);
    }
    HSTU_CUDA_OK(cudaGetLastError());
    return 0;
  });
  if (rc) return rc;
  if (want_param) {
    colsum_kernel<<<(2 * D + 31) / 32, 32 * kColsumGroups, 0, st>>>(part, grid, 2 * D, D, dw, db);
    HSTU_CUDA_OK(cudaGetLastError());
  }
  return 0;
}

#define DISPATCH_DTYPE(dt, CALL)                              \
  switch (dt) {                                               \
    case HSTU_F32: { using T = float; return CALL; }          \
    case HSTU_BF16: { using T = __nv_bfloat16; return CALL; } \
    case HSTU_F16: { using T = __half; return CALL; }         \
    default: set_error("unsupported dtype %d", dt); return HSTU_ERR_UNSUPPORTED; \
  }

int layer_norm_fwd(const void* x, const void* w, const void* b, void* y, float* mean, float* rstd, long long n, int D,
                   long long xs, long long ys, float eps, int dtype, int swish, bool rms, cudaStream_t st) {
  if (n == 0) return 0;
  if (D < 1 || D > 32 * kMaxPerLane) {
    set_error("layer_norm: D=%d outside the supported range [1, %d]", D, 32 * kMaxPerLane);
    return HSTU_ERR_UNSUPPORTED;
  }
  if (norm_fast_applicable(dtype, D) && !swish && !rms && fast_layout({x, w, b, y}, {xs, ys}))
    return layer_norm_fwd_fast(x, w, b, y, mean, rstd, n, xs, ys, eps, dtype, st);
  DISPATCH_DTYPE(dtype, (ln_fwd_t<T>(x, w, b, y, mean, rstd, n, D, xs, ys, eps, swish, rms, st)));
}

int layer_norm_bwd(const void* dy, const void* x, const void* w, const void* b, const float* mean, const float* rstd,
                   void* dx, float* dw, float* db, float* partial, long long n, int D, long long xs, long long dys,
                   long long dxs, int dtype, int swish, bool rms, cudaStream_t st) {
  if (D < 1 || D > 32 * kMaxPerLane) {
    set_error("layer_norm: D=%d outside the supported range [1, %d]", D, 32 * kMaxPerLane);
    return HSTU_ERR_UNSUPPORTED;
  }
  if (n == 0) {
    if (dw) HSTU_CUDA_OK(cudaMemsetAsync(dw, 0, sizeof(float) * D, st));
    if (db) HSTU_CUDA_OK(cudaMemsetAsync(db, 0, sizeof(float) * D, st));
    return 0;
  }
  if (norm_fast_applicable(dtype, D) && !swish && !rms && fast_layout({dy, x, w, b, dx}, {xs, dys, dxs})) {
    const bool want_param = (dw != nullptr || db != nullptr);
    if (want_param && partial == nullptr) {
      set_error("layer_norm_bwd: dw/db requested but no partial scratch given");
      return HSTU_ERR_WORKSPACE;
    }
    int grid = 0;
    if (int rc = layer_norm_bwd_fast(dy, x, w, mean, rstd, dx, want_param ? partial : nullptr, n, xs, dys, dxs, dtype, &grid, st))
      return rc;
    if (want_param) {
      colsum_kernel<<<(2 * D + 31) / 32, 32 * kColsumGroups, 0, st>>>(partial, grid, 2 * D, D, dw, db);
      HSTU_CUDA_OK(cudaGetLastError());
    }
    return 0;
  }
  DISPATCH_DTYPE(dtype, (ln_bwd_t<T>(dy, x, w, b, mean, rstd, dx, dw, db, partial, n, D, xs, dys, dxs, swish, rms, st)));
}

template <typename T>
static int nmd_fwd_t(const void* attn, const void* u, const void* w, const void* b, void* out, float* mean, float* rstd,
                     long long n, int H, int dv, long long as, long long us, float eps, float p, unsigned long long seed,
                     int silu_u, int concat, int gn, cudaStream_t st) {
  const int G = gn ? H : 1, len = gn ? dv : H * dv;
  const bool v = can_vec<T>(len, {attn, u, gn ? nullptr : w, gn ? nullptr : b, out}, {as, us});
  const int grid = norm_grid(n * G, true);
  return dispatch_shape<T>(len, v, [&]<int VV, int PL>() -> int {
    nmd_fwd_kernel<T, VV, PL><<<grid, kNormThreads, 0, st>>>((const T*)attn, (const T*)u, (const T*)w, (const T*)b,
                                                             (T*)out, mean, rstd, n, G, len, as, us, eps, p, seed, silu_u,
                                                             concat, gn);
    HSTU_CUDA_OK(cudaGetLastError());
    return 0;
  });
}

template <typename T>
static int nmd_bwd_t(const void* dout, const void* attn, const void* u, const void* w, const void* b, const float* mean,
                     const float* rstd, void* dattn, void* du, float* dw, float* db, float* partial, long long n, int H,
                     int dv, long long as, long long us, long long das, long long dus, float p, unsigned long long seed,
                     int silu_u, int concat, int gn, cudaStream_t st) {
  const int G = gn ? H : 1, len = gn ? dv : H * dv;
  const bool v = can_vec<T>(len, {dout, attn, u, gn ? nullptr : w, gn ? nullptr : b, dattn, du}, {as, us, das, dus});
  const int grid = norm_grid(n * G);
  const bool want_param = (dw != nullptr || db != nullptr);
  if (want_param && partial == nullptr) {
    set_error("norm_mul_dropout_bwd: dw/db requested but no partial scratch given");
    return HSTU_ERR_WORKSPACE;
  }
  float* part = want_param ? partial : nullptr;
  const int np = gn ? G : len;
  const size_t smem = sizeof(float) * kNormWarps * 2 * (size_t)np;
  int rc = dispatch_shape<T>(len, v, [&]<int VV, int PL>() -> int {
    HSTU_CUDA_OK(cudaFuncSetAttribute(nmd_bwd_kernel<T, VV, PL>, cudaFuncAttributeMaxDynamicSharedMemorySize, (int)smem));
    nmd_bwd_kernel<T, VV, PL><<<grid, kNormThreads, smem, st>>>((const T*)dout, (const T*)attn, (const T*)u, (const T*)w,
                                                                (const T*)b, mean, rstd, (T*)dattn, (T*)du, part, n, G,
                                                                len, as, us, das, dus, p, seed, silu_u, concat, gn);
    HSTU_CUDA_OK(cudaGetLastError());
    return 0;
  });
  if (rc) return rc;
  if (want_param) {
    colsum_kernel<<<(2 * np + 31) / 32, 32 * kColsumGroups, 0, st>>>(part, grid, 2 * np, np, dw, db);
    HSTU_CUDA_OK(cudaGetLastError());
  }
  return 0;
}

int norm_mul_dropout_fwd(const void* attn, const void* u, const void* w, const void* b, void* out, float* mean,
                         float* rstd, long long n, int H, int dv, long long as, long long us, float eps, float p,
                         unsigned long long seed, int dtype, int silu_u, int concat, int gn, cudaStream_t st) {
  if (n == 0) return 0;
  const int len = gn ? dv : H * dv;
  if (len < 1 || len > 32 * kMaxPerLane) {
    set_error("norm_mul_dropout: normalised length %d outside [1, %d]", len, 32 * kMaxPerLane);
    return HSTU_ERR_UNSUPPORTED;
  }
  if (!gn && norm_fast_applicable(dtype, len) && fast_layout({attn, u, w, b, out}, {as, us}))
    return norm_mul_dropout_fwd_fast(attn, u, w, b, out, mean, rstd, n, as, us, eps, p, seed, dtype, silu_u, concat, st);
  DISPATCH_DTYPE(dtype, (nmd_fwd_t<T>(attn, u, w, b, out, mean, rstd, n, H, dv, as, us, eps, p, seed, silu_u, concat, gn, st)));
}

int norm_mul_dropout_bwd(const void* dout, const void* attn, const void* u, const void* w, const void* b,
                         const float* mean, const float* rstd, void* dattn, void* du, float* dw, float* db,
                         float* partial, long long n, int H, int dv, long long as, long long us, long long das,
                         long long dus, float p, unsigned long long seed, int dtype, int silu_u, int concat, int gn,
                         cudaStream_t st) {
  const int len = gn ? dv : H * dv;
  const int np = gn ? H : len;
  if (len < 1 || len > 32 * kMaxPerLane) {
    set_error("norm_mul_dropout: normalised length %d outside [1, %d]", len, 32 * kMaxPerLane);
    return HSTU_ERR_UNSUPPORTED;
  }
  if (n == 0) {
    if (dw) HSTU_CUDA_OK(cudaMemsetAsync(dw, 0, sizeof(float) * np, st));
    if (db) HSTU_CUDA_OK(cudaMemsetAsync(db, 0, sizeof(float) * np, st));
    return 0;
  }
  if (!gn && norm_fast_applicable(dtype, len) && fast_layout({dout, attn, u, w, b, dattn, du}, {as, us, das, dus})) {
    const bool want_param = (dw != nullptr || db != nullptr);
    if (want_param && partial == nullptr) {
      set_error("norm_mul_dropout_bwd: dw/db requested but no partial scratch given");
      return HSTU_ERR_WORKSPACE;
    }
    int grid = 0;
    if (int rc = norm_mul_dropout_bwd_fast(dout, attn, u, w, b, mean, rstd, dattn, du, want_param ? partial : nullptr, n, as, us,
                                           das, dus, p, seed, dtype, silu_u, concat, &grid, st))
      return rc;
    if (want_param) {
      colsum_kernel<<<(2 * len + 31) / 32, 32 * kColsumGroups, 0, st>>>(partial, grid, 2 * len, len, dw, db);
      HSTU_CUDA_OK(cudaGetLastError());
    }
    return 0;
  }
  DISPATCH_DTYPE(dtype, (nmd_bwd_t<T>(dout, attn, u, w, b, mean, rstd, dattn, du, dw, db, partial, n, H, dv, as, us, das,
                                      dus, p, seed, silu_u, concat, gn, st)));
}

template <typename T>
static int silu_t(const void* x, const void* dy, void* out, long long n, int cols, long long xs, long long dys,
                  long long os, bool bwd, cudaStream_t st) {
  constexpr int VEC = 16 / sizeof(T);
  const bool v = can_vec<T>(cols, {x, dy, out}, {xs, dys, os});
  const long long total = n * (cols / (v ? VEC : 1));
  const int per_thread = (v && !bwd) ? 4 : 1;
  long long blocks = (total + 256 * per_thread - 1) / (256 * per_thread);
  const long long cap = bwd ? 132 * 16 : 132 * 8;
  if (blocks > cap) blocks = cap;
  if (blocks < 1) blocks = 1;
#define LAUNCH(VV, BB) silu_kernel<T, VV, BB><<<(int)blocks, 256, 0, st>>>((const T*)x, (const T*)dy, (T*)out, n, cols, xs, dys, os)
  if (bwd) {
    if (v) LAUNCH(VEC, true); else LAUNCH(1, true);
  } else {
    if (v) LAUNCH(VEC, false); else LAUNCH(1, false);
  }
#undef LAUNCH
  HSTU_CUDA_OK(cudaGetLastError());
  return 0;
}

int silu_fwd_bwd(const void* x, const void* dy, void* out, long long n, int cols, long long xs, long long dys,
                 long long os, int dtype, bool bwd, cudaStream_t st) {
  if (n == 0 || cols == 0) return 0;
  DISPATCH_DTYPE(dtype, (silu_t<T>(x, dy, out, n, cols, xs, dys, os, bwd, st)));
}

int norm_partial_rows() { return kPartialRows; }

}
```

generative_recommenders_b200/ops/hstu_attention.py:

```python
import ctypes as C
from typing import Optional, Tuple

import torch

from .. import _lib
from ..common import HammerKernel, require_cuda_kernel, switch_to_contiguous_if_needed


def _fill_common(p, max_seq_len, alpha, q, k, v, seq_offsets, num_targets, max_attn_len, contextual_seq_len,
                 min_full_attn_seq_len, impl, delta_q_len=0):
    if seq_offsets.dtype not in (torch.int32, torch.int64):
        raise RuntimeError("seq_offsets must be int32 or int64")
    if num_targets is not None and num_targets.dtype not in (torch.int32, torch.int64):
        raise RuntimeError("num_targets must be int32 or int64")
    p.abi_version = _lib.ABI_VERSION
    p.dtype = _lib.dtype_code(q)
    p.impl = impl
    p.batch = seq_offsets.numel() - 1
    p.heads = q.shape[1]
    p.dqk = q.shape[2]
    p.dv = v.shape[2]
    p.max_seq_len = int(max_seq_len)
    p.total_rows = k.shape[0]
    p.alpha = float(alpha)
    p.max_attn_len = int(max_attn_len)
    p.min_full_attn_seq_len = int(min_full_attn_seq_len)
    p.contextual_seq_len = int(contextual_seq_len)
    p.delta_q_len = int(delta_q_len)
    p.offsets_are_i64 = int(seq_offsets.dtype == torch.int64)
    p.num_targets_are_i64 = int(num_targets is not None and num_targets.dtype == torch.int64)
    p.seq_offsets = seq_offsets.data_ptr()
    p.num_targets = _lib.ptr(num_targets)
    p.q, p.k, p.v = q.data_ptr(), k.data_ptr(), v.data_ptr()
    p.q_row_stride, p.q_head_stride = q.stride(0), q.stride(1)
    p.k_row_stride, p.k_head_stride = k.stride(0), k.stride(1)
    p.v_row_stride, p.v_head_stride = v.stride(0), v.stride(1)


def _workspace(p, bwd: bool, device):
    nbytes = _lib.lib().hstu_attn_workspace_bytes(C.byref(p), int(bwd))
    if nbytes == 0:
        p.workspace, p.workspace_bytes = None, 0
        return None
    ws = torch.empty(nbytes + 256, dtype=torch.uint8, device=device)
    base = (ws.data_ptr() + 255) // 256 * 256
    p.workspace, p.workspace_bytes = base, nbytes
    return ws


def _prep(*ts):
    return tuple(switch_to_contiguous_if_needed(t) for t in ts)


def cuda_hstu_attention_fwd(
    max_seq_len: int, alpha: float, q: torch.Tensor, k: torch.Tensor, v: torch.Tensor, seq_offsets: torch.Tensor,
    num_targets: Optional[torch.Tensor] = None, max_attn_len: int = 0, contextual_seq_len: int = 0,
    min_full_attn_seq_len: int = 0, impl: int = _lib.IMPL_AUTO, delta_q_len: int = 0,
    out: Optional[torch.Tensor] = None, bias: Optional[Tuple[torch.Tensor, torch.Tensor, torch.Tensor]] = None,
    descales: Optional[Tuple[Optional[torch.Tensor], Optional[torch.Tensor], Optional[torch.Tensor]]] = None,
) -> torch.Tensor:
    if descales is not None or any(t.dtype == _FP8 for t in (q, k, v)):
        if bias is not None or delta_q_len:
            raise RuntimeError("fp8 attention: the relative bias and delta_q are not supported")
        return cuda_hstu_attention_fwd_fp8(max_seq_len, alpha, q, k, v, seq_offsets, descales, num_targets, max_attn_len,
                                           contextual_seq_len, min_full_attn_seq_len, impl, out)
    dev = _lib.require_cuda(q, k, v, seq_offsets, num_targets)
    q, k, v = _prep(q, k, v)
    seq_offsets = seq_offsets.contiguous()
    if num_targets is not None:
        num_targets = num_targets.contiguous()
    if out is None:
        out = torch.empty((q.shape[0], q.shape[1], v.shape[2]), dtype=v.dtype, device=dev)
    p = _lib.AttnParams()
    _fill_common(p, max_seq_len, alpha, q, k, v, seq_offsets, num_targets, max_attn_len, contextual_seq_len,
                 min_full_attn_seq_len, impl, delta_q_len)
    p.out = out.data_ptr()
    p.o_row_stride, p.o_head_stride = out.stride(0), out.stride(1)
    keep = _fill_bias(p, bias, None)
    ws = _workspace(p, False, dev)
    with torch.cuda.device(dev), _lib.timed("attn_fwd", dev):
        _lib.check(_lib.lib().hstu_attn_fwd(C.byref(p), _lib.stream_ptr(dev)), "hstu_attn_fwd")
    if delta_q_len:
        _lib.note_launch(2 if ws is not None else 1)
    else:
        _lib.note_launch(3 if ws is not None else 1)
    del ws, keep
    return out


_FP8 = torch.float8_e4m3fn


def cuda_hstu_attention_fwd_fp8(
    max_seq_len: int, alpha: float, q: torch.Tensor, k: torch.Tensor, v: torch.Tensor, seq_offsets: torch.Tensor,
    descales: Optional[Tuple[Optional[torch.Tensor], Optional[torch.Tensor], Optional[torch.Tensor]]] = None,
    num_targets: Optional[torch.Tensor] = None, max_attn_len: int = 0, contextual_seq_len: int = 0,
    min_full_attn_seq_len: int = 0, impl: int = _lib.IMPL_AUTO, out: Optional[torch.Tensor] = None,
) -> torch.Tensor:
    if not all(t.dtype == _FP8 for t in (q, k, v)):
        raise RuntimeError(f"fp8 attention: q, k and v must all be torch.float8_e4m3fn (got {q.dtype}, {k.dtype}, {v.dtype}); "
                           "descales apply to fp8 inputs only")
    dev = _lib.require_cuda(q, k, v, seq_offsets, num_targets)
    q, k, v = _prep(q, k, v)
    seq_offsets = seq_offsets.contiguous()
    if num_targets is not None:
        num_targets = num_targets.contiguous()
    B, H = seq_offsets.numel() - 1, q.shape[1]
    ds = _lib.Descales()
    for name, d in zip("qkv", descales if descales is not None else (None, None, None)):
        if d is None:
            continue
        if d.dtype != torch.float32 or tuple(d.shape) != (B, H):
            raise RuntimeError(f"fp8 attention: {name}_descale must be an fp32 [B, H] = [{B}, {H}] tensor "
                               f"(got {d.dtype} {tuple(d.shape)})")
        if d.device != dev:
            raise RuntimeError(f"fp8 attention: {name}_descale is on {d.device}, the inputs on {dev}")
        setattr(ds, name, d.data_ptr())
        setattr(ds, f"{name}_batch_stride", d.stride(0))
        setattr(ds, f"{name}_head_stride", d.stride(1))
    if out is None:
        out = torch.empty((q.shape[0], H, v.shape[2]), dtype=torch.bfloat16, device=dev)
    elif out.dtype != torch.bfloat16:
        raise RuntimeError(f"fp8 attention: out must be bf16 (got {out.dtype})")
    p = _lib.AttnParams()
    _fill_common(p, max_seq_len, alpha, q, k, v, seq_offsets, num_targets, max_attn_len, contextual_seq_len,
                 min_full_attn_seq_len, impl)
    p.out = out.data_ptr()
    p.o_row_stride, p.o_head_stride = out.stride(0), out.stride(1)
    ws = _workspace(p, False, dev)
    with torch.cuda.device(dev), _lib.timed("attn_fwd_fp8", dev):
        _lib.check(_lib.lib().hstu_attn_fwd_fp8(C.byref(p), C.byref(ds), _lib.stream_ptr(dev)), "hstu_attn_fwd_fp8")
    _lib.note_launch(2)
    del ws
    return out


def cuda_hstu_attention_bwd(
    max_seq_len: int, alpha: float, dout: torch.Tensor, q: torch.Tensor, k: torch.Tensor, v: torch.Tensor,
    dq: torch.Tensor, dk: torch.Tensor, dv: torch.Tensor, seq_offsets: torch.Tensor,
    num_targets: Optional[torch.Tensor] = None, max_attn_len: int = 0, contextual_seq_len: int = 0,
    min_full_attn_seq_len: int = 0, impl: int = _lib.IMPL_AUTO,
    bias: Optional[Tuple[torch.Tensor, torch.Tensor, torch.Tensor]] = None,
    dbias: Optional[Tuple[torch.Tensor, torch.Tensor]] = None,
    deterministic: Optional[bool] = None,
) -> None:
    if deterministic is None:
        deterministic = torch.are_deterministic_algorithms_enabled()
    dev = _lib.require_cuda(dout, q, k, v, dq, dk, dv, seq_offsets, num_targets)
    q, k, v, dout = _prep(q, k, v, dout)
    for g in (dq, dk, dv):
        if g.stride(-1) != 1:
            raise RuntimeError("dq/dk/dv must have a dense last dimension")
    seq_offsets = seq_offsets.contiguous()
    if num_targets is not None:
        num_targets = num_targets.contiguous()
    p = _lib.AttnParams()
    _fill_common(p, max_seq_len, alpha, q, k, v, seq_offsets, num_targets, max_attn_len, contextual_seq_len,
                 min_full_attn_seq_len, impl)
    p.dout, p.dq, p.dk, p.dv_out = dout.data_ptr(), dq.data_ptr(), dk.data_ptr(), dv.data_ptr()
    p.do_row_stride, p.do_head_stride = dout.stride(0), dout.stride(1)
    p.dq_row_stride, p.dq_head_stride = dq.stride(0), dq.stride(1)
    p.dk_row_stride, p.dk_head_stride = dk.stride(0), dk.stride(1)
    p.dv_row_stride, p.dv_head_stride = dv.stride(0), dv.stride(1)
    p.deterministic = int(bool(deterministic))
    keep = _fill_bias(p, bias, dbias)
    ws = _workspace(p, True, dev)
    with torch.cuda.device(dev), _lib.timed("attn_bwd", dev):
        _lib.check(_lib.lib().hstu_attn_bwd(C.byref(p), _lib.stream_ptr(dev)), "hstu_attn_bwd")
    _lib.note_launch(4 if ws is not None and p.dtype == _lib.BF16 and p.dqk == 32 else 2)
    del ws, keep


def _fill_bias(p, bias, dbias):
    if bias is None:
        return None
    pos_w, ts_w, timestamps = bias
    keep = []
    n, B = int(p.max_seq_len), int(p.batch)
    if pos_w is not None and pos_w.numel() != 2 * n - 1:
        raise RuntimeError(f"relative position bias: pos_w must have 2 * max_seq_len - 1 = {2 * n - 1} entries, got {pos_w.numel()}")
    if (ts_w is None) != (timestamps is None):
        raise RuntimeError("relative time bias: ts_w and timestamps must be given together")
    if ts_w is not None:
        if tuple(timestamps.shape) != (B, n):
            raise RuntimeError(f"relative time bias: timestamps must be [B, max_seq_len] = [{B}, {n}], got {tuple(timestamps.shape)}")
        if ts_w.numel() < 2:
            raise RuntimeError("relative time bias: ts_w must have num_buckets + 1 >= 2 entries")
    if pos_w is not None:
        pos_w = pos_w.detach().float().contiguous()
        p.pos_w = pos_w.data_ptr()
        keep.append(pos_w)
    if ts_w is not None:
        ts_w = ts_w.detach().float().contiguous()
        timestamps = timestamps.to(torch.int64).contiguous()
        p.ts_w, p.timestamps = ts_w.data_ptr(), timestamps.data_ptr()
        p.num_ts_buckets = ts_w.numel() - 1
        keep += [ts_w, timestamps]
    if dbias is not None:
        dpos_w, dts_w = dbias
        p.dpos_w = _lib.ptr(dpos_w)
        p.dts_w = _lib.ptr(dts_w)
    return keep


class _HSTUAttentionFunction(torch.autograd.Function):
    @staticmethod
    def forward(ctx, max_seq_len, alpha, q, k, v, seq_offsets, num_targets, max_attn_len, contextual_seq_len,
                min_full_attn_seq_len, impl):
        out = cuda_hstu_attention_fwd(max_seq_len, alpha, q, k, v, seq_offsets, num_targets, max_attn_len,
                                      contextual_seq_len, min_full_attn_seq_len, impl)
        ctx.save_for_backward(q, k, v, seq_offsets, num_targets)
        ctx.args = (max_seq_len, alpha, max_attn_len, contextual_seq_len, min_full_attn_seq_len, impl)
        return out

    @staticmethod
    def backward(ctx, dout):
        q, k, v, seq_offsets, num_targets = ctx.saved_tensors
        max_seq_len, alpha, max_attn_len, contextual_seq_len, min_full, impl = ctx.args
        dq = torch.empty(q.shape, dtype=q.dtype, device=q.device)
        dk = torch.empty(k.shape, dtype=k.dtype, device=k.device)
        dv = torch.empty(v.shape, dtype=v.dtype, device=v.device)
        cuda_hstu_attention_bwd(max_seq_len, alpha, dout, q, k, v, dq, dk, dv, seq_offsets, num_targets, max_attn_len,
                                contextual_seq_len, min_full, impl)
        return None, None, dq, dk, dv, None, None, None, None, None, None


def hstu_mha(
    max_seq_len: int,
    alpha: float,
    q: torch.Tensor,
    k: torch.Tensor,
    v: torch.Tensor,
    seq_offsets: torch.Tensor,
    causal: bool = True,
    dropout_pr: float = 0.0,
    training: bool = True,
    num_targets: Optional[torch.Tensor] = None,
    max_attn_len: int = 0,
    contextual_seq_len: int = 0,
    min_full_attn_seq_len: int = 0,
    sort_by_length: bool = False,
    kernel: HammerKernel = HammerKernel.CUDA,
    enable_tma: bool = False,
    impl: int = _lib.IMPL_AUTO,
) -> torch.Tensor:
    _, H, _ = q.shape
    torch._assert(max_seq_len > 0, "max_seq_len must be larger than 0")
    torch._assert(q.dim() == 3, "q must be 3-D")
    torch._assert(k.shape == q.shape, "k must be the same shape as q")
    torch._assert(v.dim() == 3, "v must be 3-D")
    torch._assert(v.shape[0] == q.shape[0], "wrong v shape[0]")
    torch._assert(v.shape[1] == H, "wrong v shape[1]")
    torch._assert(causal, "only support causal attention")
    require_cuda_kernel(kernel, "hstu_mha")
    torch._assert(dropout_pr < 1e-6, "dropout for the CUDA path is not implemented")
    return _HSTUAttentionFunction.apply(max_seq_len, alpha, q, k, v, seq_offsets, num_targets, max_attn_len,
                                        contextual_seq_len, min_full_attn_seq_len, impl)


def delta_hstu_mha(
    max_seq_len: int,
    alpha: float,
    delta_q: torch.Tensor,
    k: torch.Tensor,
    v: torch.Tensor,
    seq_offsets: torch.Tensor,
    num_targets: Optional[torch.Tensor] = None,
    max_attn_len: int = 0,
    contextual_seq_len: int = 0,
    kernel: HammerKernel = HammerKernel.CUDA,
    enable_tma: bool = False,
) -> torch.Tensor:
    L, H, D = delta_q.shape
    B = seq_offsets.size(0) - 1
    torch._assert(max_seq_len > 0, "max_seq_len must be larger than 0")
    torch._assert(delta_q.dim() == 3, "delta_q must be 3-D")
    torch._assert(L % B == 0, "delta_q must be padded")
    torch._assert(k.dim() == 3, "k must be 3-D")
    torch._assert(k.shape[1] == H, "wrong k shape[1]")
    torch._assert(k.shape[2] == D, "wrong k shape[2]")
    torch._assert(v.dim() == 3, "v must be 3-D")
    torch._assert(v.shape[1] == H, "wrong v shape[1]")
    require_cuda_kernel(kernel, "delta_hstu_mha")
    return cuda_hstu_attention_fwd(max_seq_len, alpha, delta_q, k, v, seq_offsets, num_targets, max_attn_len,
                                   contextual_seq_len, 0, _lib.IMPL_AUTO, delta_q_len=L // B)


class _RelBiasAttentionFunction(torch.autograd.Function):

    @staticmethod
    def forward(ctx, n, q, k, v, seq_offsets, pos_w, ts_w, timestamps):
        out = cuda_hstu_attention_fwd(n, 1.0, q, k, v, seq_offsets, impl=_lib.IMPL_GENERIC,
                                      bias=(pos_w, ts_w, timestamps))
        ctx.save_for_backward(q, k, v, seq_offsets, pos_w, ts_w, timestamps)
        ctx.n = n
        return out

    @staticmethod
    def backward(ctx, dout):
        q, k, v, seq_offsets, pos_w, ts_w, timestamps = ctx.saved_tensors
        dq, dk, dv = torch.empty_like(q), torch.empty_like(k), torch.empty_like(v)
        dpos = torch.zeros(pos_w.shape, dtype=torch.float32, device=q.device)
        dts = torch.zeros(ts_w.shape, dtype=torch.float32, device=q.device) if ts_w is not None else None
        cuda_hstu_attention_bwd(ctx.n, 1.0, dout, q, k, v, dq, dk, dv, seq_offsets, impl=_lib.IMPL_GENERIC,
                                bias=(pos_w, ts_w, timestamps), dbias=(dpos, dts), deterministic=False)
        return (None, dq, dk, dv, None, dpos.to(pos_w.dtype), None if dts is None else dts.to(ts_w.dtype), None)


def hstu_rel_bias_attention(n: int, q, k, v, seq_offsets, pos_w, ts_w=None, timestamps=None) -> torch.Tensor:
    return _RelBiasAttentionFunction.apply(n, q, k, v, seq_offsets, pos_w, ts_w, timestamps)
```

generative_recommenders_b200/ops/hstu_compute.py:

```python
from typing import Optional, Tuple

import torch

from .. import _lib
from ..common import HammerKernel, require_cuda_kernel
from .hstu_attention import cuda_hstu_attention_bwd, cuda_hstu_attention_fwd, hstu_mha
from .layer_norm import _partial, cuda_layer_norm_bwd, cuda_layer_norm_fwd, layer_norm


def cuda_silu_fwd(x: torch.Tensor) -> torch.Tensor:
    dev = _lib.require_cuda(x)
    n, c = x.shape
    y = torch.empty((n, c), dtype=x.dtype, device=dev)
    with torch.cuda.device(dev), _lib.timed("silu_fwd", dev):
        _lib.check(_lib.lib().hstu_silu_fwd(x.data_ptr(), y.data_ptr(), n, c, x.stride(0), y.stride(0), _lib.dtype_code(x),
                                            _lib.stream_ptr(dev)), "hstu_silu_fwd")
        _lib.note_launch(1)
    return y


def cuda_silu_bwd(dy: torch.Tensor, x: torch.Tensor, dx: torch.Tensor) -> None:
    dev = x.device
    n, c = x.shape
    dy = dy if dy.stride(-1) == 1 else dy.contiguous()
    with torch.cuda.device(dev), _lib.timed("silu_bwd", dev):
        _lib.check(_lib.lib().hstu_silu_bwd(dy.data_ptr(), x.data_ptr(), dx.data_ptr(), n, c, dy.stride(0), x.stride(0),
                                            dx.stride(0), _lib.dtype_code(x), _lib.stream_ptr(dev)), "hstu_silu_bwd")
        _lib.note_launch(1)


class _SiluFunction(torch.autograd.Function):
    @staticmethod
    def forward(ctx, x):
        ctx.save_for_backward(x)
        return cuda_silu_fwd(x)

    @staticmethod
    def backward(ctx, dy):
        (x,) = ctx.saved_tensors
        dx = torch.empty(x.shape, dtype=x.dtype, device=x.device)
        cuda_silu_bwd(dy, x, dx)
        return dx


def hstu_compute_uqvk(
    x: torch.Tensor, norm_weight: torch.Tensor, norm_bias: torch.Tensor, norm_eps: float, num_heads: int, attn_dim: int,
    hidden_dim: int, uvqk_weight: torch.Tensor, uvqk_bias: torch.Tensor, kernel: HammerKernel = HammerKernel.CUDA,
) -> Tuple[torch.Tensor, torch.Tensor, torch.Tensor, torch.Tensor]:
    require_cuda_kernel(kernel, "hstu_compute_uqvk")
    normed_x = layer_norm(x, weight=norm_weight, bias=norm_bias, eps=norm_eps, kernel=kernel)
    uvqk = torch.addmm(uvqk_bias, normed_x, uvqk_weight)
    u, v, q, k = torch.split(
        uvqk, [hidden_dim * num_heads, hidden_dim * num_heads, attn_dim * num_heads, attn_dim * num_heads], dim=1)
    u = _SiluFunction.apply(u)
    return (u, q.view(-1, num_heads, attn_dim), k.view(-1, num_heads, attn_dim), v.view(-1, num_heads, hidden_dim))


def cuda_norm_mul_dropout_fwd(attn, u, w, b, eps, p, seed, silu_u, concat_ux, group_norm, num_heads, linear_dim):
    dev = _lib.require_cuda(attn, u, w, b)
    n = attn.shape[0]
    width = num_heads * linear_dim
    out = torch.empty((n, width * (3 if concat_ux else 1)), dtype=attn.dtype, device=dev)
    nstat = n * (num_heads if group_norm else 1)
    mean = torch.empty(nstat, dtype=torch.float32, device=dev)
    rstd = torch.empty(nstat, dtype=torch.float32, device=dev)
    with torch.cuda.device(dev), _lib.timed("nmd_fwd", dev):
        _lib.check(
            _lib.lib().hstu_norm_mul_dropout_fwd(attn.data_ptr(), u.data_ptr(), w.data_ptr(), b.data_ptr(), out.data_ptr(),
                                                 mean.data_ptr(), rstd.data_ptr(), n, num_heads, linear_dim, attn.stride(0),
                                                 u.stride(0), eps, p, seed, _lib.dtype_code(attn), int(silu_u),
                                                 int(concat_ux), int(group_norm), _lib.stream_ptr(dev)),
            "hstu_norm_mul_dropout_fwd")
        _lib.note_launch(1)
    return out, mean, rstd


def cuda_norm_mul_dropout_bwd(dy, attn, u, w, b, mean, rstd, p, seed, silu_u, concat_ux, group_norm, num_heads,
                              linear_dim):
    dev = attn.device
    n = attn.shape[0]
    width = num_heads * linear_dim
    np_ = num_heads if group_norm else width
    dattn = torch.empty((n, width), dtype=attn.dtype, device=dev)
    du = torch.empty((n, width), dtype=attn.dtype, device=dev)
    dw = torch.empty(np_, dtype=torch.float32, device=dev)
    db = torch.empty(np_, dtype=torch.float32, device=dev)
    part = _partial(np_, dev)
    dy = dy.contiguous()
    with torch.cuda.device(dev), _lib.timed("nmd_bwd", dev):
        _lib.check(
            _lib.lib().hstu_norm_mul_dropout_bwd(dy.data_ptr(), attn.data_ptr(), u.data_ptr(), w.data_ptr(), b.data_ptr(),
                                                 mean.data_ptr(), rstd.data_ptr(), dattn.data_ptr(), du.data_ptr(),
                                                 dw.data_ptr(), db.data_ptr(), part.data_ptr(), n, num_heads, linear_dim,
                                                 attn.stride(0), u.stride(0), dattn.stride(0), du.stride(0), p, seed,
                                                 _lib.dtype_code(attn), int(silu_u), int(concat_ux), int(group_norm),
                                                 _lib.stream_ptr(dev)),
            "hstu_norm_mul_dropout_bwd")
        _lib.note_launch(2)
    return dattn, du, dw, db


def _next_dropout_seed(dev: torch.device, numel: int) -> int:
    gen = torch.cuda.default_generators[dev.index if dev.index is not None else torch.cuda.current_device()]
    off = gen.get_offset()
    gen.set_offset(off + ((numel + 3) // 4 + 3) // 4 * 4)
    return (gen.initial_seed() * 0x9E3779B97F4A7C15 + off * 0xD1B54A32D192ED03 + 0x2545F4914F6CDD1D) & (2**64 - 1)


def _row_major(t: torch.Tensor) -> torch.Tensor:
    return t if t.stride(-1) == 1 else t.contiguous()


class _HSTUComputeOutputFunction(torch.autograd.Function):
    @staticmethod
    def forward(ctx, attn, u, x, norm_weight, norm_bias, output_weight, eps, dropout_ratio, training, concat_ux,
                group_norm, num_heads, linear_dim, silu_u, recompute_y):
        attn, u = _row_major(attn), _row_major(u)
        w = norm_weight.to(attn.dtype).contiguous()
        b = norm_bias.to(attn.dtype).contiguous()
        p = float(dropout_ratio) if training else 0.0
        seed = _next_dropout_seed(attn.device, attn.numel() * (3 if concat_ux else 1)) if p > 0.0 else 0
        y, mean, rstd = cuda_norm_mul_dropout_fwd(attn, u, w, b, eps, p, seed, silu_u, concat_ux, group_norm, num_heads,
                                                  linear_dim)
        out = torch.addmm(x, y, output_weight.to(x.dtype))
        ctx.save_for_backward(attn, u, norm_weight, norm_bias, output_weight, mean, rstd, None if recompute_y else y)
        ctx.cfg = (eps, p, seed, silu_u, concat_ux, group_norm, num_heads, linear_dim)
        return out

    @staticmethod
    def backward(ctx, dout):
        attn, u, norm_weight, norm_bias, output_weight, mean, rstd, y = ctx.saved_tensors
        eps, p, seed, silu_u, concat_ux, group_norm, num_heads, linear_dim = ctx.cfg
        w = norm_weight.to(attn.dtype).contiguous()
        b = norm_bias.to(attn.dtype).contiguous()
        if y is None:
            y, _, _ = cuda_norm_mul_dropout_fwd(attn, u, w, b, eps, p, seed, silu_u, concat_ux, group_norm, num_heads,
                                                linear_dim)
        wo = output_weight.to(dout.dtype)
        dy = torch.mm(dout, wo.t())
        dwo = torch.mm(y.t(), dout)
        dattn, du, dw, db = cuda_norm_mul_dropout_bwd(dy, attn, u, w, b, mean, rstd, p, seed, silu_u, concat_ux,
                                                      group_norm, num_heads, linear_dim)
        return (dattn, du, dout, dw.to(norm_weight.dtype), db.to(norm_bias.dtype), dwo.to(output_weight.dtype), None, None,
                None, None, None, None, None, None, None)


def hstu_compute_output(
    attn: torch.Tensor, u: torch.Tensor, x: torch.Tensor, norm_weight: torch.Tensor, norm_bias: torch.Tensor,
    norm_eps: float, output_weight: torch.Tensor, num_heads: int, linear_dim: int, dropout_ratio: float, training: bool,
    concat_ux: bool, group_norm: bool, recompute_y_in_backward: bool, kernel: HammerKernel = HammerKernel.CUDA,
    silu_u: bool = False,
) -> torch.Tensor:
    require_cuda_kernel(kernel, "hstu_compute_output")
    return _HSTUComputeOutputFunction.apply(attn, u, x, norm_weight, norm_bias, output_weight, norm_eps, dropout_ratio,
                                            training, concat_ux, group_norm, num_heads, linear_dim, silu_u,
                                            recompute_y_in_backward)


class _HSTUPreprocessAndAttentionFunction(torch.autograd.Function):
    @staticmethod
    def forward(ctx, x, norm_weight, norm_bias, norm_eps, num_heads, attn_dim, hidden_dim, uvqk_weight, uvqk_bias,
                max_seq_len, seq_offsets, attn_alpha, num_targets, max_attn_len, contextual_seq_len, recompute_uvqk,
                recompute_normed_x, impl):
        x = _row_major(x)
        normed_x, mean, rstd = cuda_layer_norm_fwd(x, norm_weight, norm_bias, norm_eps, False)
        uvqk = torch.addmm(uvqk_bias, normed_x, uvqk_weight)
        H, dqk, dv = num_heads, attn_dim, hidden_dim
        u_pre, v, q, k = torch.split(uvqk, [dv * H, dv * H, dqk * H, dqk * H], dim=1)
        u = cuda_silu_fwd(u_pre)
        out = cuda_hstu_attention_fwd(max_seq_len, attn_alpha, q.view(-1, H, dqk), k.view(-1, H, dqk), v.view(-1, H, dv),
                                      seq_offsets, num_targets, max_attn_len, contextual_seq_len, 0, impl)
        ctx.save_for_backward(x, norm_weight, norm_bias, uvqk_weight, uvqk_bias, mean, rstd, seq_offsets, num_targets,
                              None if recompute_normed_x else normed_x,
                              None if recompute_uvqk else uvqk)
        ctx.cfg = (norm_eps, H, dqk, dv, max_seq_len, attn_alpha, max_attn_len, contextual_seq_len, impl)
        return u, out.view(-1, H * dv)

    @staticmethod
    def backward(ctx, du, dattn):
        (x, norm_weight, norm_bias, uvqk_weight, uvqk_bias, mean, rstd, seq_offsets, num_targets, normed_x,
         uvqk) = ctx.saved_tensors
        norm_eps, H, dqk, dv, max_seq_len, alpha, max_attn_len, contextual_seq_len, impl = ctx.cfg
        if normed_x is None:
            normed_x, _, _ = cuda_layer_norm_fwd(x, norm_weight, norm_bias, norm_eps, False, save_stats=False)
        if uvqk is None:
            uvqk = torch.addmm(uvqk_bias, normed_x, uvqk_weight)
        u_pre, v, q, k = torch.split(uvqk, [dv * H, dv * H, dqk * H, dqk * H], dim=1)
        duvqk = torch.empty_like(uvqk)
        d_u, d_v, d_q, d_k = torch.split(duvqk, [dv * H, dv * H, dqk * H, dqk * H], dim=1)
        dattn = _row_major(dattn)
        cuda_hstu_attention_bwd(max_seq_len, alpha, dattn.view(-1, H, dv), q.view(-1, H, dqk), k.view(-1, H, dqk),
                                v.view(-1, H, dv), d_q.view(-1, H, dqk), d_k.view(-1, H, dqk), d_v.view(-1, H, dv),
                                seq_offsets, num_targets, max_attn_len, contextual_seq_len, 0, impl)
        cuda_silu_bwd(du, u_pre, d_u)
        d_w = torch.mm(normed_x.t(), duvqk)
        d_b = duvqk.sum(dim=0)
        d_normed = torch.mm(duvqk, uvqk_weight.t())
        dx, dnw, dnb = cuda_layer_norm_bwd(d_normed, x, norm_weight, norm_bias, mean, rstd, False)
        return (dx, dnw.to(norm_weight.dtype), dnb.to(norm_bias.dtype), None, None, None, None, d_w, d_b, None, None, None,
                None, None, None, None, None, None)


def hstu_preprocess_and_attention(
    x: torch.Tensor, norm_weight: torch.Tensor, norm_bias: torch.Tensor, norm_eps: float, num_heads: int, attn_dim: int,
    hidden_dim: int, uvqk_weight: torch.Tensor, uvqk_bias: torch.Tensor, max_seq_len: int, seq_offsets: torch.Tensor,
    attn_alpha: float, causal: bool, num_targets: Optional[torch.Tensor], max_attn_len: int, contextual_seq_len: int,
    recompute_uvqk_in_backward: bool, recompute_normed_x_in_backward: bool, sort_by_length: bool, prefill: bool = False,
    kernel: HammerKernel = HammerKernel.CUDA, impl: int = _lib.IMPL_AUTO,
) -> Tuple[torch.Tensor, torch.Tensor, Optional[torch.Tensor], Optional[torch.Tensor]]:
    torch._assert(max_seq_len > 0, "max_seq_len must be larger than 0")
    torch._assert(x.dim() == 2, "x must be 2-D")
    torch._assert(x.shape[1] == uvqk_weight.shape[0], "x.shape[1] must equal uvqk_weight.shape[0]")
    torch._assert(uvqk_weight.shape[1] == 2 * num_heads * (hidden_dim + attn_dim),
                  "uvqk_weight.shape[1] must equal 2 * num_heads * (hidden_dim + attn_dim)")
    torch._assert(causal is True, "only causal attention is supported.")
    require_cuda_kernel(kernel, "hstu_preprocess_and_attention")
    if not prefill:
        u, attn_output = _HSTUPreprocessAndAttentionFunction.apply(
            x, norm_weight, norm_bias, norm_eps, num_heads, attn_dim, hidden_dim, uvqk_weight, uvqk_bias, max_seq_len,
            seq_offsets, attn_alpha, num_targets, max_attn_len, contextual_seq_len, recompute_uvqk_in_backward,
            recompute_normed_x_in_backward, impl)
        return u, attn_output, None, None
    u, q, k, v = hstu_compute_uqvk(x, norm_weight, norm_bias, norm_eps, num_heads, attn_dim, hidden_dim, uvqk_weight,
                                   uvqk_bias, kernel)
    attn_output = hstu_mha(max_seq_len=max_seq_len, alpha=attn_alpha, q=q, k=k, v=v, seq_offsets=seq_offsets, causal=causal,
                           dropout_pr=0.0, training=False, num_targets=num_targets, max_attn_len=max_attn_len,
                           contextual_seq_len=contextual_seq_len, sort_by_length=sort_by_length, kernel=kernel,
                           impl=impl).view(-1, hidden_dim * num_heads)
    return u, attn_output, k, v
```

include/hstu_b200.h:

```cpp
#ifndef HSTU_B200_H_
#define HSTU_B200_H_

#include <stddef.h>
#include <stdint.h>

#ifdef __cplusplus
extern "C" {
#endif

#define HSTU_B200_ABI_VERSION 1

typedef enum hstu_dtype { HSTU_F32 = 0, HSTU_BF16 = 1, HSTU_F16 = 2, HSTU_E4M3 = 3 } hstu_dtype;

typedef enum hstu_status {
  HSTU_OK = 0,
  HSTU_ERR_INVALID_ARGUMENT = -1,
  HSTU_ERR_UNSUPPORTED = -2,
  HSTU_ERR_CUDA = -3,
  HSTU_ERR_WORKSPACE = -4
} hstu_status;

typedef enum hstu_attn_impl {
  HSTU_IMPL_AUTO = 0,
  HSTU_IMPL_GENERIC = 1,
  HSTU_IMPL_UMMA = 2
} hstu_attn_impl;

typedef struct hstu_attn_params {
  int32_t abi_version;
  int32_t dtype;
  int32_t impl;
  int32_t batch;
  int32_t heads;
  int32_t dqk;
  int32_t dv;
  int32_t max_seq_len;
  int64_t total_rows;
  float alpha;
  int32_t max_attn_len;
  int32_t min_full_attn_seq_len;
  int32_t contextual_seq_len;
  int32_t delta_q_len;
  int32_t offsets_are_i64;
  int32_t num_targets_are_i64;
  const void* seq_offsets;
  const void* num_targets;
  const void* q;
  const void* k;
  const void* v;
  void* out;
  int64_t q_row_stride, q_head_stride;
  int64_t k_row_stride, k_head_stride;
  int64_t v_row_stride, v_head_stride;
  int64_t o_row_stride, o_head_stride;
  const void* dout;
  void* dq;
  void* dk;
  void* dv_out;
  int64_t do_row_stride, do_head_stride;
  int64_t dq_row_stride, dq_head_stride;
  int64_t dk_row_stride, dk_head_stride;
  int64_t dv_row_stride, dv_head_stride;
  const float* pos_w;
  const float* ts_w;
  const int64_t* timestamps;
  int32_t num_ts_buckets;
  int32_t deterministic;
  float* dpos_w;
  float* dts_w;
  void* workspace;
  size_t workspace_bytes;
} hstu_attn_params;

const char* hstu_last_error(void);
int hstu_abi_version(void);

size_t hstu_attn_workspace_bytes(const hstu_attn_params* p, int is_backward);
int hstu_attn_fwd(const hstu_attn_params* p, void* cuda_stream);
int hstu_attn_bwd(const hstu_attn_params* p, void* cuda_stream);

typedef struct hstu_attn_descales {
  const float* q;
  const float* k;
  const float* v;
  int64_t q_batch_stride, q_head_stride;
  int64_t k_batch_stride, k_head_stride;
  int64_t v_batch_stride, v_head_stride;
} hstu_attn_descales;
int hstu_attn_fwd_fp8(const hstu_attn_params* p, const hstu_attn_descales* descales, void* cuda_stream);
int hstu_attn_select_impl(const hstu_attn_params* p, int is_backward);

int hstu_mask_valid(int32_t len, int32_t num_targets , int32_t max_attn_len,
                    int32_t min_full_attn_seq_len, int32_t contextual_seq_len, int32_t i, int32_t j);
int hstu_kv_range_for_q_rows(int32_t len, int32_t num_targets, int32_t max_attn_len, int32_t min_full_attn_seq_len,
                             int32_t contextual_seq_len, int32_t m0, int32_t m1, int32_t* lo, int32_t* hi);
int hstu_q_range_for_kv_rows(int32_t len, int32_t num_targets, int32_t max_attn_len, int32_t min_full_attn_seq_len,
                             int32_t contextual_seq_len, int32_t n0, int32_t n1, int32_t* lo, int32_t* hi,
                             int32_t* ctx_hi);

int hstu_layer_norm_fwd(const void* x, const void* w, const void* b, void* y, float* mean, float* rstd,
                        int64_t n_rows, int32_t D, int64_t x_row_stride, int64_t y_row_stride, float eps,
                        int32_t dtype, int32_t swish, void* cuda_stream);
int hstu_layer_norm_bwd(const void* dy, const void* x, const void* w, const void* b, const float* mean,
                        const float* rstd, void* dx, float* dw, float* db, float* partial, int64_t n_rows,
                        int32_t D, int64_t x_row_stride, int64_t dy_row_stride, int64_t dx_row_stride,
                        int32_t dtype, int32_t swish, void* cuda_stream);
int32_t hstu_norm_bwd_partial_rows(void);
int hstu_rms_norm_fwd(const void* x, const void* w, void* y, float* rstd, int64_t n_rows, int32_t D, float eps,
                      int32_t dtype, void* cuda_stream);
int hstu_rms_norm_bwd(const void* dy, const void* x, const void* w, const float* rstd, void* dx, float* dw,
                      float* partial, int64_t n_rows, int32_t D, int32_t dtype, void* cuda_stream);

int hstu_norm_mul_dropout_fwd(const void* attn, const void* u, const void* w, const void* b, void* out, float* mean,
                              float* rstd, int64_t n_rows, int32_t heads, int32_t dv, int64_t attn_row_stride,
                              int64_t u_row_stride, float eps, float dropout_p, uint64_t seed, int32_t dtype,
                              int32_t silu_u, int32_t concat_ux, int32_t group_norm, void* cuda_stream);
int hstu_norm_mul_dropout_bwd(const void* dout, const void* attn, const void* u, const void* w, const void* b,
                              const float* mean, const float* rstd, void* dattn, void* du, float* dw, float* db,
                              float* partial, int64_t n_rows, int32_t heads, int32_t dv, int64_t attn_row_stride,
                              int64_t u_row_stride, int64_t dattn_row_stride, int64_t du_row_stride, float dropout_p,
                              uint64_t seed, int32_t dtype, int32_t silu_u, int32_t concat_ux, int32_t group_norm,
                              void* cuda_stream);

int hstu_silu_fwd(const void* x, void* y, int64_t n_rows, int32_t n_cols, int64_t x_row_stride, int64_t y_row_stride,
                  int32_t dtype, void* cuda_stream);
int hstu_silu_bwd(const void* dy, const void* x, void* dx, int64_t n_rows, int32_t n_cols, int64_t dy_row_stride,
                  int64_t x_row_stride, int64_t dx_row_stride, int32_t dtype, void* cuda_stream);

int hstu_jagged_concat(const void* left, const void* right, void* out, const void* offsets_left,
                       const void* offsets_right, int32_t offsets_are_i64, int32_t batch, int32_t dense_len_left,
                       int32_t dense_len_right, int32_t n_prefix, int32_t D, int32_t elem_bytes, int32_t max_seq_len,
                       void* cuda_stream);
int hstu_jagged_split(const void* in, void* left, void* right, const void* offsets_left, const void* offsets_right,
                      int32_t offsets_are_i64, int32_t batch, int32_t dense_len_left, int32_t dense_len_right,
                      int32_t n_prefix, int32_t D, int32_t elem_bytes, int32_t max_seq_len, void* cuda_stream);

int hstu_position_embeddings_fwd(const void* seq_embeddings, void* out, const float* pos_w, const float* ts_w,
                                 const void* seq_offsets, const void* seq_lengths, const void* num_targets,
                                 const int64_t* timestamps, int32_t* pos_inds, int32_t* ts_inds, int64_t total_rows,
                                 int32_t batch, int32_t D, int32_t max_pos_ind, int32_t num_time_buckets,
                                 int32_t max_contextual_seq_len, float alpha, int32_t interleave_targets,
                                 int32_t log_time_bucket, int32_t offsets_are_i64, int32_t lengths_are_i64,
                                 int32_t num_targets_are_i64, int32_t dtype, void* cuda_stream);
int hstu_position_embeddings_bwd(const void* dout, void* d_seq_embeddings, float* d_pos_w, float* d_ts_w,
                                 const int32_t* pos_inds, const int32_t* ts_inds, int64_t total_rows, int32_t D, float alpha,
                                 int32_t dtype, void* cuda_stream);

int hstu_jagged_dense_bmm_broadcast_add(const void* jagged, const void* dense, const void* bias, void* out,
                                        const void* seq_offsets, int32_t offsets_are_i64, int32_t batch, int32_t K, int32_t N,
                                        int32_t max_seq_len, int32_t dense_is_transposed, int32_t dtype, void* cuda_stream);
int hstu_jagged_dense_bmm_wgrad(const void* jagged, const void* dout, void* d_dense, void* d_bias, const void* seq_offsets,
                                int32_t offsets_are_i64, int32_t batch, int32_t K, int32_t N, int32_t max_seq_len, int32_t dtype,
                                void* cuda_stream);

typedef struct hstu_ssl_params {
  int32_t abi_version;
  int32_t dtype;
  int64_t N;
  int32_t R;
  int32_t D;
  int32_t l2_norm;
  float l2_eps;
  float temperature;
  int32_t reserved0;
  const void* q;
  const void* pos_emb;
  const void* table;
  const int64_t* pos_ids;
  const int64_t* neg_ids;
  float* logits;
  float* rnorm;
  float* lse;
  float* loss_rows;
  const float* row_coef;
  void* d_q;
  void* d_pos_emb;
  float* d_table;
} hstu_ssl_params;
int hstu_sampled_softmax_fwd(const hstu_ssl_params* p, void* cuda_stream);
int hstu_sampled_softmax_bwd(const hstu_ssl_params* p, void* cuda_stream);

#ifdef __cplusplus
}
#endif
#endif
```

Measured before the change: 103.1.

## Fuse SiLU and fp16 operand conversion into one split pass using analytic amax bounds

Adds a path for bf16 d=32 attention on sm90 that replaces the per-sequence amax reduction with an analytic bound computed from the layernorm and projection weights. A single split kernel then writes silu(u) and scaled fp16 copies of q, k and v straight from the uvqk buffer. The backward fuses the SiLU gradient with the column-sum used for the bias gradient. This removes the amax pass, the separate SiLU launch and the reduction, but the weight-derived bound is looser than a measured amax, which may cost fp16 precision.

```diff
diff --git a/generative_recommenders_b200/_lib.py b/generative_recommenders_b200/_lib.py
--- a/generative_recommenders_b200/_lib.py
+++ b/generative_recommenders_b200/_lib.py
@@ -32,7 +32,7 @@
         ("dv_row_stride", C.c_int64), ("dv_head_stride", C.c_int64),
         ("pos_w", C.c_void_p), ("ts_w", C.c_void_p), ("timestamps", C.c_void_p), ("num_ts_buckets", C.c_int32),
         ("deterministic", C.c_int32), ("dpos_w", C.c_void_p), ("dts_w", C.c_void_p),
-        ("workspace", C.c_void_p), ("workspace_bytes", C.c_size_t),
+        ("workspace", C.c_void_p), ("workspace_bytes", C.c_size_t), ("operands_prepared", C.c_int32),
     ]
 
 
@@ -66,6 +66,7 @@
     "hstu_attn_bwd": (C.c_int, [C.POINTER(AttnParams), _vp]),
     "hstu_attn_fwd_fp8": (C.c_int, [C.POINTER(AttnParams), C.POINTER(Descales), _vp]),
     "hstu_attn_select_impl": (C.c_int, [C.POINTER(AttnParams), C.c_int]),
+    "hstu_stu_attn_operands": (C.c_int, [C.POINTER(AttnParams), _i32, _vp, _i64, _vp, _vp, _vp, _vp, _i32, _vp, _i64, _vp]),
     "hstu_mask_valid": (C.c_int, [_i32] * 7),
     "hstu_kv_range_for_q_rows": (C.c_int, [_i32] * 7 + [C.POINTER(_i32)] * 2),
     "hstu_q_range_for_kv_rows": (C.c_int, [_i32] * 7 + [C.POINTER(_i32)] * 3),
@@ -78,6 +79,7 @@
     "hstu_norm_mul_dropout_bwd": (C.c_int, [_vp] * 12 + [_i64, _i32, _i32, _i64, _i64, _i64, _i64, _f32, _u64, _i32, _i32, _i32, _i32, _vp]),
     "hstu_silu_fwd": (C.c_int, [_vp, _vp, _i64, _i32, _i64, _i64, _i32, _vp]),
     "hstu_silu_bwd": (C.c_int, [_vp, _vp, _vp, _i64, _i32, _i64, _i64, _i64, _i32, _vp]),
+    "hstu_silu_bwd_colsum": (C.c_int, [_vp, _vp, _vp, _i64, _i32, _i32, _i64, _i64, _i64, _vp, _vp, _i32, _vp]),
     "hstu_jagged_concat": (C.c_int, [_vp] * 5 + [_i32] * 8 + [_vp]),
     "hstu_jagged_split": (C.c_int, [_vp] * 5 + [_i32] * 8 + [_vp]),
     "hstu_position_embeddings_fwd": (C.c_int, [_vp] * 10 + [_i64, _i32, _i32, _i32, _i32, _i32, _f32, _i32, _i32, _i32, _i32, _i32, _i32, _vp]),
diff --git a/generative_recommenders_b200/csrc/api.cu b/generative_recommenders_b200/csrc/api.cu
--- a/generative_recommenders_b200/csrc/api.cu
+++ b/generative_recommenders_b200/csrc/api.cu
@@ -141,8 +141,48 @@
   return 0;
 }
 
+static int check_prepared(const hstu_attn_params* p, bool bwd) {
+  HSTU_CHECK_ARG(p->operands_prepared == 0 || p->operands_prepared == 1, "operands_prepared must be 0 or 1 (got %d)",
+                 p->operands_prepared);
+  if (!p->operands_prepared || p->batch == 0 || p->total_rows == 0) return 0;
+  if (p->dtype != HSTU_BF16 || p->dqk != 32 || p->dv != 32 || p->delta_q_len != 0 || p->pos_w || p->ts_w ||
+      select_impl(p, bwd) != HSTU_IMPL_UMMA) {
+    set_error("prepared operands: bf16 with dqk == dv == 32 on the wgmma path only, without delta_q or a relative bias "
+              "(dtype=%d dqk=%d dv=%d delta=%d impl=%d)", p->dtype, p->dqk, p->dv, p->delta_q_len, p->impl);
+    return HSTU_ERR_UNSUPPORTED;
+  }
+  return 0;
+}
+
+int hstu_stu_attn_operands(const hstu_attn_params* p, int32_t is_backward, const void* uvqk, int64_t uvqk_row_stride,
+                           const void* norm_weight, const void* norm_bias, const void* uvqk_weight, const void* uvqk_beta,
+                           int32_t embedding_dim, void* u_out, int64_t u_row_stride, void* stream) {
+  const bool bwd = is_backward != 0;
+  if (int e = validate_attn(p, bwd)) return e;
+  HSTU_CHECK_ARG(p->operands_prepared == 1, "hstu_stu_attn_operands: p->operands_prepared must be 1");
+  if (int e = check_prepared(p, bwd)) return e;
+  HSTU_CHECK_ARG(p->batch > 0 || p->total_rows == 0, "hstu_stu_attn_operands: rows without a sequence (batch = 0)");
+  if (p->total_rows == 0) return 0;
+  const long long H = p->heads;
+  const uint16_t* base = static_cast<const uint16_t*>(uvqk);
+  HSTU_CHECK_ARG(uvqk && norm_weight && norm_bias && uvqk_weight && uvqk_beta && embedding_dim > 0,
+                 "hstu_stu_attn_operands: NULL parameter or embedding_dim <= 0");
+  HSTU_CHECK_ARG(aligned_view(uvqk, uvqk_row_stride, 8) && uvqk_row_stride >= 128 * H,
+                 "hstu_stu_attn_operands: uvqk needs a 16-byte aligned base and a row stride >= 128 H, a multiple of 8");
+  HSTU_CHECK_ARG(p->v == base + 32 * H && p->q == base + 64 * H && p->k == base + 96 * H && p->q_row_stride == uvqk_row_stride &&
+                 p->k_row_stride == uvqk_row_stride && p->v_row_stride == uvqk_row_stride && p->q_head_stride == 32 &&
+                 p->k_head_stride == 32 && p->v_head_stride == 32,
+                 "hstu_stu_attn_operands: p->q, p->k, p->v must be the q, k, v views of uvqk = [u | v | q | k]");
+  HSTU_CHECK_ARG(bwd == (u_out == nullptr), "hstu_stu_attn_operands: u_out is required in the forward and NULL in the backward");
+  if (!bwd) HSTU_CHECK_ARG(aligned_view(u_out, u_row_stride, 8), "hstu_stu_attn_operands: u_out needs 16-byte aligned rows");
+  if (int e = bind_device(uvqk)) return e;
+  const StuOperandsArgs a{uvqk, uvqk_row_stride, norm_weight, norm_bias, uvqk_weight, uvqk_beta, embedding_dim, u_out, u_row_stride};
+  return stu_operands_prepare(*p, bwd, a, (cudaStream_t)stream);
+}
+
 int hstu_attn_fwd(const hstu_attn_params* p, void* stream) {
   if (int e = validate_attn(p, false)) return e;
+  if (int e = check_prepared(p, false)) return e;
   HSTU_CHECK_ARG(p->dtype != HSTU_E4M3, "hstu_attn_fwd: fp8 (e4m3) inputs go through hstu_attn_fwd_fp8 (with their descales)");
   if (p->batch == 0 || p->total_rows == 0) return 0;
   if (int e = bind_device(p->q)) return e;
@@ -154,6 +194,7 @@
 
 int hstu_attn_bwd(const hstu_attn_params* p, void* stream) {
   if (int e = validate_attn(p, true)) return e;
+  if (int e = check_prepared(p, true)) return e;
   if (p->dtype == HSTU_E4M3) {
     set_error("hstu_attn_bwd: fp8 (e4m3) attention has no backward (hstu_attn_fwd_fp8 is forward only)");
     return HSTU_ERR_UNSUPPORTED;
@@ -169,6 +210,7 @@
 int hstu_attn_fwd_fp8(const hstu_attn_params* p, const hstu_attn_descales* descales, void* stream) {
   if (int e = validate_attn(p, false)) return e;
   HSTU_CHECK_ARG(p->dtype == HSTU_E4M3, "hstu_attn_fwd_fp8: q, k, v must be HSTU_E4M3 (got dtype %d)", p->dtype);
+  HSTU_CHECK_ARG(p->operands_prepared == 0, "hstu_attn_fwd_fp8: operands_prepared is for bf16 attention at d = 32");
   if (int e = validate_descales(descales)) return e;
   const int impl = select_impl(p, false);
   if (impl < 0) return impl;
@@ -287,6 +329,16 @@
   HSTU_CHECK_ARG(n_rows >= 0 && (n_rows == 0 || (dy && x && dx)), "silu_bwd: NULL argument");
   return silu_fwd_bwd(x, dy, dx, n_rows, n_cols, x_row_stride, dy_row_stride, dx_row_stride, dtype, true,
                       (cudaStream_t)stream);
+}
+
+int hstu_silu_bwd_colsum(const void* dy, const void* x, void* g, int64_t n_rows, int32_t u_cols, int32_t g_cols,
+                         int64_t dy_row_stride, int64_t x_row_stride, int64_t g_row_stride, float* partial, float* col_sum,
+                         int32_t dtype, void* stream) {
+  HSTU_CHECK_ARG(n_rows >= 0 && u_cols >= 0 && g_cols >= u_cols, "silu_bwd_colsum: bad sizes");
+  HSTU_CHECK_ARG(partial && col_sum && (n_rows == 0 || (dy && x && g)), "silu_bwd_colsum: NULL argument");
+  if (int e = bind_device(col_sum)) return e;
+  return silu_bwd_colsum(dy, x, g, n_rows, u_cols, g_cols, dy_row_stride, x_row_stride, g_row_stride, partial, col_sum, dtype,
+                         (cudaStream_t)stream);
 }
 
 int hstu_jagged_concat(const void* left, const void* right, void* out, const void* offsets_left, const void* offsets_right,
diff --git a/generative_recommenders_b200/csrc/attn_fp16_operands.cu b/generative_recommenders_b200/csrc/attn_fp16_operands.cu
--- a/generative_recommenders_b200/csrc/attn_fp16_operands.cu
+++ b/generative_recommenders_b200/csrc/attn_fp16_operands.cu
@@ -1,4 +1,6 @@
+#include <cuda_bf16.h>
 #include <cuda_fp16.h>
+#include <float.h>
 #include <cuda_fp8.h>
 #include <string.h>
 
@@ -18,7 +20,7 @@
 
 struct PreParams {
   PreOperand op[kAmaxSlots];
-  int nops;
+  int first, nops;
   const void* seq_offsets;
   int offsets_i64, max_seq_len, heads;
   int d;
@@ -37,7 +39,7 @@
   const int rows = min(kPreRows, len - r0);
   __shared__ uint32_t red[kAmaxSlots][kPreThreads / 32];
   const int warp = threadIdx.x >> 5, lane = threadIdx.x & 31;
-  for (int o = 0; o < p.nops; ++o) {
+  for (int o = p.first; o < p.nops; ++o) {
     const PreOperand& op = p.op[o];
     uint32_t m = 0u;
     for (int c = threadIdx.x; c < rows * 4; c += kPreThreads) {
@@ -56,7 +58,7 @@
     if (lane == 0) red[o][warp] = m;
   }
   __syncthreads();
-  if (threadIdx.x < p.nops) {
+  if (threadIdx.x >= p.first && threadIdx.x < p.nops) {
     uint32_t m = 0u;
 #pragma unroll
     for (int w = 0; w < kPreThreads / 32; ++w) m = max(m, red[threadIdx.x][w]);
@@ -78,7 +80,7 @@
     const OperandExps ex = operand_exps(p.amax + ((long long)b * p.heads + h) * kAmaxSlots, p.alpha, kPreD);
     exps[0] = ex.q, exps[1] = ex.k, exps[2] = ex.v, exps[3] = ex.o;
   }
-  for (int o = 0; o < p.nops; ++o) {
+  for (int o = p.first; o < p.nops; ++o) {
     const PreOperand& op = p.op[o];
     const int e = exps[o];
     for (int c = threadIdx.x; c < rows * cpr; c += kPreThreads) {
@@ -109,6 +111,123 @@
   }
 }
 
+constexpr double kStuMargin = 1.0 + 1.0 / 32;
+constexpr int kStuD = 32, kStuRows = 32, kStuUnroll = 4;
+
+struct StuBoundParams {
+  const uint16_t *ln_w, *ln_b, *w, *beta;
+  int D, heads, batch;
+  uint32_t* amax;
+};
+
+__host__ __device__ inline int stu_column(int slot, int h, int heads) {
+  return (slot == kAmaxV ? 1 : slot + 2) * kStuD * heads + h * kStuD;
+}
+
+__global__ void __launch_bounds__(kPreThreads) stu_operand_bound_kernel(const __grid_constant__ StuBoundParams p) {
+  const int h = blockIdx.x, slot = blockIdx.y, warp = threadIdx.x >> 5, lane = threadIdx.x & 31;
+  const int ncols = 4 * kStuD * p.heads, col = stu_column(slot, h, p.heads) + lane;
+  double sq = 0.0, ab = 0.0;
+  bool finite = true;
+  for (int k = warp; k < p.D; k += kPreThreads / 32) {
+    const float w = bf16_bits_to_float(p.ln_w[k]), b = bf16_bits_to_float(p.ln_b[k]);
+    const float x = bf16_bits_to_float(p.w[(long long)k * ncols + col]);
+    finite = finite && isfinite(w) && isfinite(b) && isfinite(x);
+    const double wx = (double)w * x;
+    sq += wx * wx;
+    ab += fabs((double)b * x);
+  }
+  __shared__ double red[2][kPreThreads / 32][32];
+  __shared__ int bad[kPreThreads / 32];
+  __shared__ uint32_t bits;
+  red[0][warp][lane] = sq;
+  red[1][warp][lane] = ab;
+  const int any_bad = __any_sync(0xffffffffu, !finite);
+  if (lane == 0) bad[warp] = any_bad;
+  __syncthreads();
+  if (warp == 0) {
+    sq = 0.0, ab = 0.0;
+    int nonfinite = 0;
+#pragma unroll
+    for (int i = 0; i < kPreThreads / 32; ++i) sq += red[0][i][lane], ab += red[1][i][lane], nonfinite |= bad[i];
+    const float beta = bf16_bits_to_float(p.beta[col]);
+    nonfinite |= __any_sync(0xffffffffu, !isfinite(beta));
+    double bound = (sqrt((double)p.D * sq) + ab + fabs((double)beta)) * kStuMargin;
+#pragma unroll
+    for (int s = 16; s > 0; s >>= 1) bound = fmax(bound, __shfl_xor_sync(0xffffffffu, bound, s));
+    if (lane == 0) bits = nonfinite ? 0x7f800000u : __float_as_uint(bound > FLT_MAX ? FLT_MAX : __double2float_ru(bound));
+  }
+  __syncthreads();
+  for (int b = threadIdx.x; b < p.batch; b += kPreThreads) {
+    uint32_t* a = p.amax + ((long long)b * p.heads + h) * kAmaxSlots;
+    a[slot] = bits;
+    if (slot == kAmaxQ) a[kAmaxDO] = 0u;
+  }
+}
+
+struct StuSplitParams {
+  const uint16_t* uvqk;
+  long long row_stride, rows;
+  int heads;
+  uint16_t* u_out;
+  long long u_row_stride;
+  __half* dst[3];
+  const uint32_t* amax;
+  float alpha;
+};
+
+__global__ void __launch_bounds__(kPreThreads) stu_operand_split_kernel(const __grid_constant__ StuSplitParams p) {
+  extern __shared__ int s_exp[];
+  for (int h = threadIdx.x; h < p.heads; h += kPreThreads) {
+    const OperandExps ex = operand_exps(p.amax + (long long)h * kAmaxSlots, p.alpha, kPreD);
+    s_exp[h * 3 + kAmaxQ] = ex.q, s_exp[h * 3 + kAmaxK] = ex.k, s_exp[h * 3 + kAmaxV] = ex.v;
+  }
+  __syncthreads();
+  const long long row0 = (long long)blockIdx.x * kStuRows;
+  const int rows = (int)min((long long)kStuRows, p.rows - row0);
+  const int cph = kStuD / 8, cpb = cph * p.heads;
+  const int c0 = p.u_out ? 0 : cpb, cpr = 4 * cpb - c0, n = rows * cpr;
+  for (int i0 = threadIdx.x; i0 < n; i0 += kPreThreads * kStuUnroll) {
+    uint4 x[kStuUnroll];
+    long long row[kStuUnroll];
+    int col[kStuUnroll];
+#pragma unroll
+    for (int u = 0; u < kStuUnroll; ++u) {
+      const int i = i0 + u * kPreThreads;
+      if (i < n) {
+        const int r = i / cpr;
+        row[u] = row0 + r;
+        col[u] = (i - r * cpr + c0) * 8;
+        x[u] = *reinterpret_cast<const uint4*>(p.uvqk + row[u] * p.row_stride + col[u]);
+      }
+    }
+#pragma unroll
+    for (int u = 0; u < kStuUnroll; ++u) {
+      if (i0 + u * kPreThreads >= n) continue;
+      const uint32_t w[4] = {x[u].x, x[u].y, x[u].z, x[u].w};
+      uint32_t y[4];
+      const int blk = col[u] / (kStuD * p.heads), c = col[u] - blk * kStuD * p.heads, h = c / kStuD;
+      if (blk == 0) {
+#pragma unroll
+        for (int i = 0; i < 4; ++i) {
+          const __nv_bfloat16 lo = __float2bfloat16_rn(silu_f(bf16_bits_to_float(w[i] & 0xffffu)));
+          const __nv_bfloat16 hi = __float2bfloat16_rn(silu_f(bf16_bits_to_float(w[i] >> 16)));
+          y[i] = (uint32_t)__bfloat16_as_ushort(lo) | ((uint32_t)__bfloat16_as_ushort(hi) << 16);
+        }
+        *reinterpret_cast<uint4*>(p.u_out + row[u] * p.u_row_stride + c) = make_uint4(y[0], y[1], y[2], y[3]);
+      } else {
+        const int slot = blk == 1 ? kAmaxV : blk - 2, e = s_exp[h * 3 + slot];
+#pragma unroll
+        for (int i = 0; i < 4; ++i) {
+          const __half2 v = __floats2half2_rn(scalbnf(bf16_bits_to_float(w[i] & 0xffffu), e), scalbnf(bf16_bits_to_float(w[i] >> 16), e));
+          y[i] = *reinterpret_cast<const uint32_t*>(&v);
+        }
+        *reinterpret_cast<uint4*>(p.dst[slot] + (row[u] * p.heads + h) * kStuD + (c - h * kStuD)) = make_uint4(y[0], y[1], y[2], y[3]);
+      }
+    }
+  }
+}
+
 static size_t align256(size_t n) { return (n + 255) / 256 * 256; }
 
 size_t fp16_operands_workspace_bytes(const hstu_attn_params& p, bool bwd) {
@@ -117,7 +236,7 @@
   return amax + (bwd ? 4 : 3) * copy;
 }
 
-int fp16_operands_prepass(const hstu_attn_params& p, bool bwd, Fp16Operands* out, cudaStream_t st) {
+static int fp16_operands_layout(const hstu_attn_params& p, bool bwd, PreParams* pp, Fp16Operands* out) {
   const size_t need = fp16_operands_workspace_bytes(p, bwd);
   if (p.workspace == nullptr || p.workspace_bytes < need) {
     set_error("hstu_attn_%s: workspace of %zu bytes required (got %zu)", bwd ? "bwd" : "fwd", need, p.workspace_bytes);
@@ -126,27 +245,29 @@
   uint8_t* ws = reinterpret_cast<uint8_t*>(p.workspace);
   const size_t amax_bytes = (size_t)p.batch * p.heads * kAmaxSlots * sizeof(uint32_t);
   const size_t copy = align256((size_t)p.total_rows * p.heads * kPreD * sizeof(__half));
-  PreParams pp;
-  memset(&pp, 0, sizeof(pp));
-  pp.amax = reinterpret_cast<uint32_t*>(ws);
+  memset(pp, 0, sizeof(*pp));
+  pp->amax = reinterpret_cast<uint32_t*>(ws);
   const void* src[kAmaxSlots] = {p.q, p.k, p.v, p.dout};
   const long long rs[kAmaxSlots] = {p.q_row_stride, p.k_row_stride, p.v_row_stride, p.do_row_stride};
   const long long hs[kAmaxSlots] = {p.q_head_stride, p.k_head_stride, p.v_head_stride, p.do_head_stride};
-  pp.nops = bwd ? 4 : 3;
-  for (int o = 0; o < pp.nops; ++o) {
-    pp.op[o].src = src[o];
-    pp.op[o].row_stride = rs[o];
-    pp.op[o].head_stride = hs[o];
-    pp.op[o].dst = reinterpret_cast<__half*>(ws + align256(amax_bytes) + o * copy);
-    out->copy[o] = pp.op[o].dst;
-  }
-  out->amax = pp.amax;
-  pp.seq_offsets = p.seq_offsets;
-  pp.offsets_i64 = p.offsets_are_i64;
-  pp.max_seq_len = p.max_seq_len;
-  pp.heads = p.heads;
-  pp.alpha = p.alpha;
-  HSTU_CUDA_OK(cudaMemsetAsync(pp.amax, 0, amax_bytes, st));
+  pp->nops = bwd ? 4 : 3;
+  for (int o = 0; o < pp->nops; ++o) {
+    pp->op[o].src = src[o];
+    pp->op[o].row_stride = rs[o];
+    pp->op[o].head_stride = hs[o];
+    pp->op[o].dst = reinterpret_cast<__half*>(ws + align256(amax_bytes) + o * copy);
+    out->copy[o] = pp->op[o].dst;
+  }
+  out->amax = pp->amax;
+  pp->seq_offsets = p.seq_offsets;
+  pp->offsets_i64 = p.offsets_are_i64;
+  pp->max_seq_len = p.max_seq_len;
+  pp->heads = p.heads;
+  pp->alpha = p.alpha;
+  return 0;
+}
+
+static int fp16_operands_amax_convert(const hstu_attn_params& p, const PreParams& pp, cudaStream_t st) {
   if (p.batch == 0 || p.max_seq_len <= 0) return 0;
   const dim3 grid((p.max_seq_len + kPreRows - 1) / kPreRows, p.heads, p.batch);
   fp16_operands_amax_kernel<<<grid, kPreThreads, 0, st>>>(pp);
@@ -154,6 +275,52 @@
   fp16_operands_convert_kernel<false><<<grid, kPreThreads, 0, st>>>(pp);
   HSTU_CUDA_OK(cudaGetLastError());
   return 0;
+}
+
+int fp16_operands_prepass(const hstu_attn_params& p, bool bwd, Fp16Operands* out, cudaStream_t st) {
+  PreParams pp;
+  if (int e = fp16_operands_layout(p, bwd, &pp, out)) return e;
+  HSTU_CUDA_OK(cudaMemsetAsync(pp.amax, 0, (size_t)p.batch * p.heads * kAmaxSlots * sizeof(uint32_t), st));
+  return fp16_operands_amax_convert(p, pp, st);
+}
+
+int fp16_operands_prepared(const hstu_attn_params& p, bool bwd, Fp16Operands* out) {
+  PreParams pp;
+  return fp16_operands_layout(p, bwd, &pp, out);
+}
+
+int stu_operands_prepare(const hstu_attn_params& p, bool bwd, const StuOperandsArgs& a, cudaStream_t st) {
+  PreParams pp;
+  Fp16Operands f16;
+  if (int e = fp16_operands_layout(p, bwd, &pp, &f16)) return e;
+  if (p.batch == 0 || p.total_rows == 0) return 0;
+  StuBoundParams bp;
+  bp.ln_w = static_cast<const uint16_t*>(a.norm_weight);
+  bp.ln_b = static_cast<const uint16_t*>(a.norm_bias);
+  bp.w = static_cast<const uint16_t*>(a.uvqk_weight);
+  bp.beta = static_cast<const uint16_t*>(a.uvqk_beta);
+  bp.D = a.embedding_dim;
+  bp.heads = p.heads;
+  bp.batch = p.batch;
+  bp.amax = pp.amax;
+  stu_operand_bound_kernel<<<dim3(p.heads, 3), kPreThreads, 0, st>>>(bp);
+  HSTU_CUDA_OK(cudaGetLastError());
+  StuSplitParams sp;
+  sp.uvqk = static_cast<const uint16_t*>(a.uvqk);
+  sp.row_stride = a.uvqk_row_stride;
+  sp.rows = p.total_rows;
+  sp.heads = p.heads;
+  sp.u_out = static_cast<uint16_t*>(a.u_out);
+  sp.u_row_stride = a.u_row_stride;
+  for (int o = 0; o < 3; ++o) sp.dst[o] = pp.op[o].dst;
+  sp.amax = pp.amax;
+  sp.alpha = p.alpha;
+  const long long blocks = (p.total_rows + kStuRows - 1) / kStuRows;
+  stu_operand_split_kernel<<<(unsigned)blocks, kPreThreads, 3 * p.heads * sizeof(int), st>>>(sp);
+  HSTU_CUDA_OK(cudaGetLastError());
+  if (!bwd) return 0;
+  pp.first = kAmaxDO;
+  return fp16_operands_amax_convert(p, pp, st);
 }
 
 size_t e4m3_v_copy_bytes(const hstu_attn_params& p) { return align256((size_t)p.total_rows * p.heads * p.dv * sizeof(__half)); }
diff --git a/generative_recommenders_b200/csrc/attn_wgmma_bwd.cu b/generative_recommenders_b200/csrc/attn_wgmma_bwd.cu
--- a/generative_recommenders_b200/csrc/attn_wgmma_bwd.cu
+++ b/generative_recommenders_b200/csrc/attn_wgmma_bwd.cu
@@ -110,7 +110,7 @@
     case 32: {
       if (!bf) return launch_bwd_wgmma<32, false, true>(p, st);
       Fp16Operands f16;
-      if (int e = fp16_operands_prepass(p, true, &f16, st)) return e;
+      if (int e = p.operands_prepared ? fp16_operands_prepared(p, true, &f16) : fp16_operands_prepass(p, true, &f16, st)) return e;
       return launch_bwd_wgmma<32, false, true>(p, st, &f16);
     }
     case 64:
diff --git a/generative_recommenders_b200/csrc/attn_wgmma_fwd.cu b/generative_recommenders_b200/csrc/attn_wgmma_fwd.cu
--- a/generative_recommenders_b200/csrc/attn_wgmma_fwd.cu
+++ b/generative_recommenders_b200/csrc/attn_wgmma_fwd.cu
@@ -104,7 +104,7 @@
     case 32: {
       if (!bf) return launch_fwd<32, false>(p, st);
       Fp16Operands f16;
-      if (int e = fp16_operands_prepass(p, false, &f16, st)) return e;
+      if (int e = p.operands_prepared ? fp16_operands_prepared(p, false, &f16) : fp16_operands_prepass(p, false, &f16, st)) return e;
       return launch_fwd<32, false>(p, st, &f16);
     }
     case 64: return bf ? launch_fwd<64, true>(p, st) : launch_fwd<64, false>(p, st);
diff --git a/generative_recommenders_b200/csrc/internal.h b/generative_recommenders_b200/csrc/internal.h
--- a/generative_recommenders_b200/csrc/internal.h
+++ b/generative_recommenders_b200/csrc/internal.h
@@ -26,6 +26,16 @@
 };
 size_t fp16_operands_workspace_bytes(const hstu_attn_params& p, bool bwd);
 int fp16_operands_prepass(const hstu_attn_params& p, bool bwd, Fp16Operands* out, cudaStream_t st);
+int fp16_operands_prepared(const hstu_attn_params& p, bool bwd, Fp16Operands* out);
+struct StuOperandsArgs {
+  const void* uvqk;
+  long long uvqk_row_stride;
+  const void *norm_weight, *norm_bias, *uvqk_weight, *uvqk_beta;
+  int embedding_dim;
+  void* u_out;
+  long long u_row_stride;
+};
+int stu_operands_prepare(const hstu_attn_params& p, bool bwd, const StuOperandsArgs& a, cudaStream_t st);
 size_t e4m3_v_copy_bytes(const hstu_attn_params& p);
 int e4m3_v_prepass(const hstu_attn_params& p, const void** v16, cudaStream_t st);
 
@@ -50,6 +60,8 @@
 int silu_fwd_bwd(const void* x, const void* dy, void* out, long long n, int cols, long long xs, long long dys,
                  long long os, int dtype, bool bwd, cudaStream_t st);
 int norm_partial_rows();
+int silu_bwd_colsum(const void* dy, const void* x, void* g, long long n, int ucols, int gcols, long long dys, long long xs,
+                    long long gs, float* partial, float* colsum, int dtype, cudaStream_t st);
 
 struct PosArgs {
   const void* seq;
diff --git a/generative_recommenders_b200/csrc/norm.cu b/generative_recommenders_b200/csrc/norm.cu
--- a/generative_recommenders_b200/csrc/norm.cu
+++ b/generative_recommenders_b200/csrc/norm.cu
@@ -535,6 +535,55 @@
   }
 }
 
+constexpr int kColsumThreads = 128, kColsumUnroll = 4;
+
+template <typename T>
+__global__ void __launch_bounds__(kColsumThreads) silu_bwd_colsum_kernel(const T* __restrict__ dy, const T* __restrict__ x,
+                                                                          T* __restrict__ g, long long n_rows, int ucols,
+                                                                          int gcols, long long dys, long long xs, long long gs,
+                                                                          float* __restrict__ partial) {
+  constexpr int VEC = 16 / sizeof(T);
+  const long long r0 = n_rows * blockIdx.x / gridDim.x, r1 = n_rows * (blockIdx.x + 1) / gridDim.x;
+  for (int col = threadIdx.x * VEC; col < gcols; col += kColsumThreads * VEC) {
+    const bool is_u = col < ucols;
+    float acc[VEC];
+#pragma unroll
+    for (int i = 0; i < VEC; ++i) acc[i] = 0.f;
+    for (long long rb = r0; rb < r1; rb += kColsumUnroll) {
+      T gv[kColsumUnroll][VEC], xv[kColsumUnroll][VEC];
+#pragma unroll
+      for (int k = 0; k < kColsumUnroll; ++k) {
+        const long long r = rb + k;
+        if (r >= r1) continue;
+        if (is_u) {
+          *reinterpret_cast<uint4*>(gv[k]) = *reinterpret_cast<const uint4*>(dy + r * dys + col);
+          *reinterpret_cast<uint4*>(xv[k]) = *reinterpret_cast<const uint4*>(x + r * xs + col);
+        } else {
+          *reinterpret_cast<uint4*>(gv[k]) = *reinterpret_cast<const uint4*>(g + r * gs + col);
+        }
+      }
+#pragma unroll
+      for (int k = 0; k < kColsumUnroll; ++k) {
+        const long long r = rb + k;
+        if (r >= r1) continue;
+        if (is_u) {
+#pragma unroll
+          for (int i = 0; i < VEC; ++i) {
+            const float xf = Cvt<T>::to_f(xv[k][i]);
+            const float sg = sigmoid_f(xf);
+            gv[k][i] = Cvt<T>::from_f(Cvt<T>::to_f(gv[k][i]) * sg * (1.f + xf * (1.f - sg)));
+          }
+          *reinterpret_cast<uint4*>(g + r * gs + col) = *reinterpret_cast<const uint4*>(gv[k]);
+        }
+#pragma unroll
+        for (int i = 0; i < VEC; ++i) acc[i] += Cvt<T>::to_f(gv[k][i]);
+      }
+    }
+#pragma unroll
+    for (int i = 0; i < VEC; ++i) partial[(long long)blockIdx.x * gcols + col + i] = acc[i];
+  }
+}
+
 static inline bool aligned16(const void* p) { return p == nullptr || (reinterpret_cast<uintptr_t>(p) & 15) == 0; }
 
 static inline int norm_grid(long long n_vec, bool fwd = false) {
@@ -803,4 +852,25 @@
 
 int norm_partial_rows() { return kPartialRows; }
 
-}
+template <typename T>
+static int silu_bwd_colsum_t(const void* dy, const void* x, void* g, long long n, int ucols, int gcols, long long dys,
+                             long long xs, long long gs, float* partial, float* colsum, cudaStream_t st) {
+  constexpr int VEC = 16 / sizeof(T);
+  if (ucols % VEC || gcols % VEC || ucols > gcols || !can_vec<T>(gcols, {dy, x, g}, {dys, xs, gs})) {
+    set_error("silu_bwd_colsum: 16-byte aligned rows and column counts that are multiples of %d required", VEC);
+    return HSTU_ERR_UNSUPPORTED;
+  }
+  silu_bwd_colsum_kernel<T><<<kPartialRows, kColsumThreads, 0, st>>>((const T*)dy, (const T*)x, (T*)g, n, ucols, gcols, dys,
+                                                                      xs, gs, partial);
+  HSTU_CUDA_OK(cudaGetLastError());
+  colsum_kernel<<<(gcols + 31) / 32, 32 * kColsumGroups, 0, st>>>(partial, kPartialRows, gcols, gcols, colsum, nullptr);
+  HSTU_CUDA_OK(cudaGetLastError());
+  return 0;
+}
+
+int silu_bwd_colsum(const void* dy, const void* x, void* g, long long n, int ucols, int gcols, long long dys, long long xs,
+                    long long gs, float* partial, float* colsum, int dtype, cudaStream_t st) {
+  DISPATCH_DTYPE(dtype, (silu_bwd_colsum_t<T>(dy, x, g, n, ucols, gcols, dys, xs, gs, partial, colsum, st)));
+}
+
+}
diff --git a/generative_recommenders_b200/ops/hstu_attention.py b/generative_recommenders_b200/ops/hstu_attention.py
--- a/generative_recommenders_b200/ops/hstu_attention.py
+++ b/generative_recommenders_b200/ops/hstu_attention.py
@@ -52,12 +52,25 @@
     return tuple(switch_to_contiguous_if_needed(t) for t in ts)
 
 
+StuOperands = Tuple[torch.Tensor, torch.Tensor, torch.Tensor, torch.Tensor, torch.Tensor, Optional[torch.Tensor]]
+
+
+def _prepare_stu_operands(p, bwd: bool, stu: StuOperands, dev) -> None:
+    uvqk, norm_weight, norm_bias, uvqk_weight, uvqk_bias, u_out = stu
+    p.operands_prepared = 1
+    _lib.check(_lib.lib().hstu_stu_attn_operands(
+        C.byref(p), int(bwd), uvqk.data_ptr(), uvqk.stride(0), norm_weight.data_ptr(), norm_bias.data_ptr(),
+        uvqk_weight.data_ptr(), uvqk_bias.data_ptr(), uvqk_weight.shape[0], _lib.ptr(u_out),
+        0 if u_out is None else u_out.stride(0), _lib.stream_ptr(dev)), "hstu_stu_attn_operands")
+
+
 def cuda_hstu_attention_fwd(
     max_seq_len: int, alpha: float, q: torch.Tensor, k: torch.Tensor, v: torch.Tensor, seq_offsets: torch.Tensor,
     num_targets: Optional[torch.Tensor] = None, max_attn_len: int = 0, contextual_seq_len: int = 0,
     min_full_attn_seq_len: int = 0, impl: int = _lib.IMPL_AUTO, delta_q_len: int = 0,
     out: Optional[torch.Tensor] = None, bias: Optional[Tuple[torch.Tensor, torch.Tensor, torch.Tensor]] = None,
     descales: Optional[Tuple[Optional[torch.Tensor], Optional[torch.Tensor], Optional[torch.Tensor]]] = None,
+    stu_operands: Optional[StuOperands] = None,
 ) -> torch.Tensor:
     if descales is not None or any(t.dtype == _FP8 for t in (q, k, v)):
         if bias is not None or delta_q_len:
@@ -79,9 +92,13 @@
     keep = _fill_bias(p, bias, None)
     ws = _workspace(p, False, dev)
     with torch.cuda.device(dev), _lib.timed("attn_fwd", dev):
+        if stu_operands is not None:
+            _prepare_stu_operands(p, False, stu_operands, dev)
         _lib.check(_lib.lib().hstu_attn_fwd(C.byref(p), _lib.stream_ptr(dev)), "hstu_attn_fwd")
     if delta_q_len:
         _lib.note_launch(2 if ws is not None else 1)
+    elif stu_operands is not None:
+        _lib.note_launch(3 if ws is not None else 0)
     else:
         _lib.note_launch(3 if ws is not None else 1)
     del ws, keep
@@ -143,6 +160,7 @@
     bias: Optional[Tuple[torch.Tensor, torch.Tensor, torch.Tensor]] = None,
     dbias: Optional[Tuple[torch.Tensor, torch.Tensor]] = None,
     deterministic: Optional[bool] = None,
+    stu_operands: Optional[StuOperands] = None,
 ) -> None:
     if deterministic is None:
         deterministic = torch.are_deterministic_algorithms_enabled()
@@ -166,8 +184,15 @@
     keep = _fill_bias(p, bias, dbias)
     ws = _workspace(p, True, dev)
     with torch.cuda.device(dev), _lib.timed("attn_bwd", dev):
+        if stu_operands is not None:
+            _prepare_stu_operands(p, True, stu_operands, dev)
         _lib.check(_lib.lib().hstu_attn_bwd(C.byref(p), _lib.stream_ptr(dev)), "hstu_attn_bwd")
-    _lib.note_launch(4 if ws is not None and p.dtype == _lib.BF16 and p.dqk == 32 else 2)
+    if ws is None:
+        _lib.note_launch(0 if stu_operands is not None else 2)
+    elif stu_operands is not None:
+        _lib.note_launch(6)
+    else:
+        _lib.note_launch(4 if p.dtype == _lib.BF16 and p.dqk == 32 else 2)
     del ws, keep
 
 
diff --git a/generative_recommenders_b200/ops/hstu_compute.py b/generative_recommenders_b200/ops/hstu_compute.py
--- a/generative_recommenders_b200/ops/hstu_compute.py
+++ b/generative_recommenders_b200/ops/hstu_compute.py
@@ -27,6 +27,21 @@
         _lib.check(_lib.lib().hstu_silu_bwd(dy.data_ptr(), x.data_ptr(), dx.data_ptr(), n, c, dy.stride(0), x.stride(0),
                                             dx.stride(0), _lib.dtype_code(x), _lib.stream_ptr(dev)), "hstu_silu_bwd")
         _lib.note_launch(1)
+
+
+def cuda_silu_bwd_colsum(dy: torch.Tensor, x: torch.Tensor, g: torch.Tensor) -> torch.Tensor:
+    dev = x.device
+    n, c = x.shape
+    if dy.stride(-1) != 1 or dy.data_ptr() % 16 or dy.stride(0) % 8:
+        dy = dy.clone(memory_format=torch.contiguous_format)
+    part = torch.empty(_lib.lib().hstu_norm_bwd_partial_rows() * g.shape[1], dtype=torch.float32, device=dev)
+    out = torch.empty(g.shape[1], dtype=torch.float32, device=dev)
+    with torch.cuda.device(dev), _lib.timed("silu_bwd", dev):
+        _lib.check(_lib.lib().hstu_silu_bwd_colsum(dy.data_ptr(), x.data_ptr(), g.data_ptr(), n, c, g.shape[1], dy.stride(0),
+                                                   x.stride(0), g.stride(0), part.data_ptr(), out.data_ptr(),
+                                                   _lib.dtype_code(x), _lib.stream_ptr(dev)), "hstu_silu_bwd_colsum")
+        _lib.note_launch(2)
+    return out
 
 
 class _SiluFunction(torch.autograd.Function):
@@ -157,6 +172,12 @@
                                             recompute_y_in_backward)
 
 
+def _stu_operands_apply(uvqk, params, H, dqk, dv, impl, seq_offsets) -> bool:
+    return (dqk == 32 and dv == 32 and impl != _lib.IMPL_GENERIC and seq_offsets.numel() > 1
+            and all(t.dtype == torch.bfloat16 for t in (uvqk,) + params)
+            and torch.cuda.get_device_capability(uvqk.device)[0] == 9)
+
+
 class _HSTUPreprocessAndAttentionFunction(torch.autograd.Function):
     @staticmethod
     def forward(ctx, x, norm_weight, norm_bias, norm_eps, num_heads, attn_dim, hidden_dim, uvqk_weight, uvqk_bias,
@@ -167,9 +188,16 @@
         uvqk = torch.addmm(uvqk_bias, normed_x, uvqk_weight)
         H, dqk, dv = num_heads, attn_dim, hidden_dim
         u_pre, v, q, k = torch.split(uvqk, [dv * H, dv * H, dqk * H, dqk * H], dim=1)
-        u = cuda_silu_fwd(u_pre)
+        params = tuple(t.contiguous() for t in (norm_weight, norm_bias, uvqk_weight, uvqk_bias))
+        stu = None
+        if _stu_operands_apply(uvqk, params, H, dqk, dv, impl, seq_offsets):
+            u = torch.empty(u_pre.shape, dtype=uvqk.dtype, device=uvqk.device)
+            stu = (uvqk,) + params + (u,)
+        else:
+            u = cuda_silu_fwd(u_pre)
         out = cuda_hstu_attention_fwd(max_seq_len, attn_alpha, q.view(-1, H, dqk), k.view(-1, H, dqk), v.view(-1, H, dv),
-                                      seq_offsets, num_targets, max_attn_len, contextual_seq_len, 0, impl)
+                                      seq_offsets, num_targets, max_attn_len, contextual_seq_len, 0, impl,
+                                      stu_operands=stu)
         ctx.save_for_backward(x, norm_weight, norm_bias, uvqk_weight, uvqk_bias, mean, rstd, seq_offsets, num_targets,
                               None if recompute_normed_x else normed_x,
                               None if recompute_uvqk else uvqk)
@@ -189,12 +217,17 @@
         duvqk = torch.empty_like(uvqk)
         d_u, d_v, d_q, d_k = torch.split(duvqk, [dv * H, dv * H, dqk * H, dqk * H], dim=1)
         dattn = _row_major(dattn)
+        params = tuple(t.contiguous() for t in (norm_weight, norm_bias, uvqk_weight, uvqk_bias))
+        stu = (uvqk,) + params + (None,) if _stu_operands_apply(uvqk, params, H, dqk, dv, impl, seq_offsets) else None
         cuda_hstu_attention_bwd(max_seq_len, alpha, dattn.view(-1, H, dv), q.view(-1, H, dqk), k.view(-1, H, dqk),
                                 v.view(-1, H, dv), d_q.view(-1, H, dqk), d_k.view(-1, H, dqk), d_v.view(-1, H, dv),
-                                seq_offsets, num_targets, max_attn_len, contextual_seq_len, 0, impl)
-        cuda_silu_bwd(du, u_pre, d_u)
+                                seq_offsets, num_targets, max_attn_len, contextual_seq_len, 0, impl, stu_operands=stu)
+        if stu is not None:
+            d_b = cuda_silu_bwd_colsum(du, u_pre, duvqk).to(duvqk.dtype)
+        else:
+            cuda_silu_bwd(du, u_pre, d_u)
+            d_b = duvqk.sum(dim=0)
         d_w = torch.mm(normed_x.t(), duvqk)
-        d_b = duvqk.sum(dim=0)
         d_normed = torch.mm(duvqk, uvqk_weight.t())
         dx, dnw, dnb = cuda_layer_norm_bwd(d_normed, x, norm_weight, norm_bias, mean, rstd, False)
         return (dx, dnw.to(norm_weight.dtype), dnb.to(norm_bias.dtype), None, None, None, None, d_w, d_b, None, None, None,
diff --git a/include/hstu_b200.h b/include/hstu_b200.h
--- a/include/hstu_b200.h
+++ b/include/hstu_b200.h
@@ -70,6 +70,7 @@
   float* dts_w;
   void* workspace;
   size_t workspace_bytes;
+  int32_t operands_prepared;
 } hstu_attn_params;
 
 const char* hstu_last_error(void);
@@ -78,6 +79,10 @@
 size_t hstu_attn_workspace_bytes(const hstu_attn_params* p, int is_backward);
 int hstu_attn_fwd(const hstu_attn_params* p, void* cuda_stream);
 int hstu_attn_bwd(const hstu_attn_params* p, void* cuda_stream);
+
+int hstu_stu_attn_operands(const hstu_attn_params* p, int32_t is_backward, const void* uvqk, int64_t uvqk_row_stride,
+                           const void* norm_weight, const void* norm_bias, const void* uvqk_weight, const void* uvqk_beta,
+                           int32_t embedding_dim, void* u_out, int64_t u_row_stride, void* cuda_stream);
 
 typedef struct hstu_attn_descales {
   const float* q;
@@ -126,6 +131,9 @@
                   int32_t dtype, void* cuda_stream);
 int hstu_silu_bwd(const void* dy, const void* x, void* dx, int64_t n_rows, int32_t n_cols, int64_t dy_row_stride,
                   int64_t x_row_stride, int64_t dx_row_stride, int32_t dtype, void* cuda_stream);
+int hstu_silu_bwd_colsum(const void* dy, const void* x, void* g, int64_t n_rows, int32_t u_cols, int32_t g_cols,
+                         int64_t dy_row_stride, int64_t x_row_stride, int64_t g_row_stride, float* partial, float* col_sum,
+                         int32_t dtype, void* cuda_stream);
 
 int hstu_jagged_concat(const void* left, const void* right, void* out, const void* offsets_left,
                        const void* offsets_right, int32_t offsets_are_i64, int32_t batch, int32_t dense_len_left,
```

After: 105.3, median of 6. 2.1% higher.
